# XinMing0411/AC-VAE

Hardware: AMD Instinct MI355X
Metric: train-step captions/s (and audio-sec/s) at B=32, 1/2/4/8 MI355X (higher is better)
Workload: dtype f32

## Files before the change

### acvae_amd/csrc/conv.h

```cpp
#pragma once
#include <hip/hip_runtime.h>
#include <stdint.h>
#include "common.h"
#include "job_table.h"

struct DropoutSpec {
  float p;
  const uint8_t* mask;
  uint64_t seed;
  uint32_t site;
};

enum { UP_PLAIN = 0, UP_POOL = 1, UP_DROP = 2 };

namespace acvae {
int conv3x3_igemm(const float* X, const float* scale, const float* shift, const float* Wp, float* Y, float* partials,
                  int N, int H, int W, int Cin, int Cout, hipStream_t st);
int conv_partials_rows(int N, int H, int W);
int conv3x3_igemm_bf16(const bf16_t* X, const float* scale, const float* shift, const bf16_t* Wp, bf16_t* Y,
                       float* partials, int N, int H, int W, int Cin, int Cout, hipStream_t st);
long conv3x3_wgrad_bf16_slab_floats(int N, int H, int W, int Cin, int Cout);
int conv3x3_wgrad_bf16_splits(int N, int H, int W, int Cin, int Cout);
int conv3x3_wgrad_bf16_launch(const bf16_t* dY, const bf16_t* X, const float* scale, const float* shift, float* slab, int N,
                              int H, int W, int Cin, int Cout, hipStream_t st);
int wgrad_reduce(const float* slab, int nsplit, float* dW_oihw, int Cout, int Cin, hipStream_t st);
long conv3x3_wgrad_slab_floats(int N, int H, int W, int Cin, int Cout);
int conv3x3_wgrad(const float* dY, const float* X, const float* scale, const float* shift, float* dW_oihw, float* slab,
                  int N, int H, int W, int Cin, int Cout, hipStream_t st);
bool conv3x3_wino_ok(int H, int W, int Cin, int Cout);
long conv3x3_wino_weight_floats(int Cin, int Cout);
int conv_wino_partials_rows(int N, int H, int W);
int conv3x3_wino_weights(const float* W_oihw, float* U, int Cout, int Cin, bool dgrad, hipStream_t st);
struct WinoWeightsJob { const float* W; float* U; int Cout, Cin, dgrad; };
using WinoWeightsBatch = RangeTable<WinoWeightsJob, 32>;
int conv3x3_wino_weights_batch(WinoWeightsBatch& b, hipStream_t st);
struct WinoBnReduce { const float* Y; const float* scale; const float* shift; const float* mean; const float* invstd; };
int conv3x3_wino(const float* X, const float* scale, const float* shift, const float* U, float* Y, float* partials, int N,
                 int H, int W, int Cin, int Cout, hipStream_t st, const WinoBnReduce* red = nullptr);
bool conv3x3_wino_wgrad_ok(int H, int W, int Cin, int Cout);
long conv3x3_wino_wgrad_slab_floats(int N, int H, int W, int Cin, int Cout);
int conv3x3_wino_wgrad(const float* dY, const float* X, const float* scale, const float* shift, float* dW_oihw, float* slab,
                       int N, int H, int W, int Cin, int Cout, hipStream_t st);
template <class T>
int repack_weights(const float* W_oihw, T* Wf, T* Wd, int Cout, int Cin, hipStream_t st);
struct RepackJob { const float* W; void* dst; int Cout, Cin, dgrad; };
using RepackBatch = RangeTable<RepackJob, 32>;
template <class T>
int repack_weights_batch(RepackBatch& b, hipStream_t st);
inline int conv3x3_igemm(const bf16_t* X, const float* scale, const float* shift, const bf16_t* Wp, bf16_t* Y,
                         float* partials, int N, int H, int W, int Cin, int Cout, hipStream_t st) {
  return conv3x3_igemm_bf16(X, scale, shift, Wp, Y, partials, N, H, W, Cin, Cout, st);
}
inline int conv3x3_wgrad(const bf16_t* dY, const bf16_t* X, const float* scale, const float* shift, float* dW_oihw,
                         float* slab, int N, int H, int W, int Cin, int Cout, hipStream_t st) {
  int r = conv3x3_wgrad_bf16_launch(dY, X, scale, shift, slab, N, H, W, Cin, Cout, st);
  if (r != 0) return r;
  return wgrad_reduce(slab, conv3x3_wgrad_bf16_splits(N, H, W, Cin, Cout), dW_oihw, Cout, Cin, st);
}
template <class T>
inline long conv3x3_wgrad_slab_floats_t(int N, int H, int W, int Cin, int Cout) {
  return sizeof(T) == 2 ? conv3x3_wgrad_bf16_slab_floats(N, H, W, Cin, Cout) : conv3x3_wgrad_slab_floats(N, H, W, Cin, Cout);
}
int bn0_stats(const float* x, float* partials, long rows, int F, int* nparts, hipStream_t st);
int bn0_partials_rows(long rows);
int bn_finalize(const float* partials, int P, int C, double count, const float* gamma, const float* beta,
                float* running_mean, float* running_var, int64_t* nbt, int training, float* scale, float* shift,
                float* mean, float* invstd, double* dpart, hipStream_t st);
long colsum_scratch_doubles(int width);
int colsum_tickets_reset(double* dpart, hipStream_t st);
long colsum_ticket_words();
int colsum2(const float* x, int P, int width, double* dpart, float* out, float* out2, int split, hipStream_t st);
struct ColsumJob { const float* x; int P, width; float* out; float* out_b; int R; long d0; };
using ColsumBatch = RangeTable<ColsumJob, 6, int>;
int colsum_batch(ColsumBatch& b, double* dpart, long dpart_doubles, hipStream_t st);
bool colsum_batch_plan(ColsumBatch& b, long dpart_doubles, long* dsum_doubles);
int conv1_first_blocks(int N, int T);
template <class TY>
int conv1_first_fwd(const float* x, const float* scale0, const float* shift0, const float* W1, TY* Y,
                    float* partials, int N, int T, int F, hipStream_t st);
template <class TY>
int conv1_first_bwd(const float* x, const float* scale0, const float* shift0, const float* mean0, const float* invstd0,
                    const float* W1, const TY* dY, float* dw_part, float* bn_part, float* dW1, float* dgamma0,
                    float* dbeta0, double* dpart, int N, int T, int F, hipStream_t st);
template <class T>
int bn_relu_pool(const T* Y, const float* scale, const float* shift, T* P, int N, int H, int W, int C,
                 DropoutSpec drop, hipStream_t st, bool pool = true);
int bn_bwd_blocks(int N, int H, int W, int C);
template <class T>
int bn_bwd(const T* Y, const T* dO, int upstream, const float* scale, const float* shift, const float* mean,
           const float* invstd, float* partials, float* sum_g, float* sum_gy, T* dY, double* dpart, int N, int H,
           int W, int C, DropoutSpec drop, hipStream_t st, bool batch_stats = true, int ready_rows = 0);
template <class T>
int relu_mask(const T* Y, const float* scale, const float* shift, uint8_t* out, int N, int H, int W, int C, hipStream_t st);
template <class T>
int freq_mean(const T* P, float* out, long rows, int Fp, int C, hipStream_t st);
template <class T>
int freq_mean_bwd(const float* dae, T* dP, long rows, int Fp, int C, hipStream_t st);
int time_pool(const float* ae, float* out, int N, int S, int C, DropoutSpec drop, hipStream_t st);
int relu_dropout(float* x, int total, DropoutSpec drop, hipStream_t st);
}

int acvae_gemm_nt_dual(const float* A1, int64_t lda1, const float* B1, int64_t ldb1, int K1, const float* A2,
                       int64_t lda2, const float* B2, int64_t ldb2, int K2, const float* bias, float* C, int64_t ldc,
                       int M, int N, int accumulate, hipStream_t st, float* skws = nullptr);
int acvae_gemm_nt_pair(const float* A0, int64_t lda0, const float* B0, int64_t ldb0, int K0, const float* bias0, float* C0,
                       int64_t ldc0, int N0, int acc0, const float* A1, int64_t lda1, const float* B1, int64_t ldb1, int K1,
                       const float* bias1, float* C1, int64_t ldc1, int N1, int acc1, int M, hipStream_t st);
constexpr int TN_TICKETS = 256;
int acvae_gemm_tn_fused(const float* A, int64_t lda, const float* B, int64_t ldb, float* C, int64_t ldc, int M, int N, int K,
                        int accumulate, float* ws, int64_t ws_bytes, hipStream_t st);
long acvae_skinny_ws_floats();
long acvae_skinny_ticket_words();
int acvae_skinny_ws_reset(float* ws, hipStream_t st);
struct TransposeJob { const float* in; long ld_in; float* out; long ld_out; int rows, cols; };
using TransposeBatch = acvae::RangeTable<TransposeJob, 12, int>;
int acvae_transpose_batch(TransposeBatch& b, hipStream_t st);
```

### acvae_amd/csrc/conv.hip

```cpp
#include "mfma_tile.h"
#include "../../include/acvae_hip.h"
#include "conv.h"
#include "prof.h"

namespace {
using namespace mfma;

struct FastDiv {
  unsigned long long mul;
  static FastDiv make(int d) { return FastDiv{((1ULL << 40) + (unsigned long long)d - 1) / (unsigned long long)d}; }
  __device__ __forceinline__ int div(int x) const { return (int)(((unsigned long long)(unsigned)x * mul) >> 40); }
};

struct ConvKMajorLoader {
  const float* X;
  const float* scale;
  const float* shift;
  int H, W, C, M, NC;
  FastDiv dW, dH;
  int dy, dx, ci;
  bool colok;
  float4 sc, sh;
  template <int WT>
  __device__ __forceinline__ void init(int col0) {
// ... 422 lines not shown
        acc[0][1] = __builtin_amdgcn_mfma_f32_32x32x2f32(af.x, bp.y, acc[0][1], 0, 0, 0);
        acc[0][2] = __builtin_amdgcn_mfma_f32_32x32x2f32(af.x, bc, acc[0][2], 0, 0, 0);
        acc[1][0] = __builtin_amdgcn_mfma_f32_32x32x2f32(af.y, bp.x, acc[1][0], 0, 0, 0);
        acc[1][1] = __builtin_amdgcn_mfma_f32_32x32x2f32(af.y, bp.y, acc[1][1], 0, 0, 0);
        acc[1][2] = __builtin_amdgcn_mfma_f32_32x32x2f32(af.y, bc, acc[1][2], 0, 0, 0);
      }
    }
    if (ks + 1 < nk) stash(cur ^ 1);
    __syncthreads();
  }
  float* Cw = EM == 2 ? Cs : slab + (long)(2 * z + wm) * Cout * NC;
#pragma unroll
  for (int em = 0; em < 2; ++em)
#pragma unroll
    for (int r = 0; r < 16; ++r) {
      const int rho = (r & 3) + 8 * (r >> 2) + 4 * lh;
      const int m = row0 + (EM == 2 ? wm * 64 : 0) + 2 * rho + em;
      if (m >= Cout) continue;
      float* out = Cw + (long)m * NC + dyi * 3 * C + c0;
      out[2 * wn * C + 2 * li + 0] = acc[em][0][r];
      out[2 * wn * C + 2 * li + 1] = acc[em][1][r];
      out[C + wn * 32 + li] = acc[em][2][r];
    }
}

__global__ void wgrad_reduce_kernel(const float* __restrict__ slab, int nsplit, float* __restrict__ dW, int Cout,
                                    int Cin) {
  const long total = (long)Cout * 9 * Cin;
  for (long i = blockIdx.x * (long)blockDim.x + threadIdx.x; i < total; i += (long)gridDim.x * blockDim.x) {
    float a0 = 0.f, a1 = 0.f, a2 = 0.f, a3 = 0.f;
    int z = 0;
    for (; z + 3 < nsplit; z += 4) {
      a0 += slab[(long)z * total + i]; a1 += slab[(long)(z + 1) * total + i];
      a2 += slab[(long)(z + 2) * total + i]; a3 += slab[(long)(z + 3) * total + i];
    }
    for (; z < nsplit; ++z) a0 += slab[(long)z * total + i];
    const float acc = (a0 + a1) + (a2 + a3);
    const int co = (int)(i / (9 * Cin)), rem = (int)(i % (9 * Cin));
    const int tap = rem / Cin, ci = rem % Cin;
    dW[((long)co * Cin + ci) * 9 + tap] = acc;
  }
}

template <class T>
__global__ void repack_fwd_kernel(const float* __restrict__ W, T* __restrict__ Wf, int Cout, int Cin) {
  const long total = (long)Cout * Cin * 9;
  for (long i = blockIdx.x * (long)blockDim.x + threadIdx.x; i < total; i += (long)gridDim.x * blockDim.x) {
    const int co = (int)(i / (9 * Cin)), rem = (int)(i % (9 * Cin));
    const int tap = rem / Cin, ci = rem % Cin;
    Wf[i] = (T)W[((long)co * Cin + ci) * 9 + tap];
  }
}
template <class T>
__global__ void repack_dgrad_kernel(const float* __restrict__ W, T* __restrict__ Wd, int Cout, int Cin) {
  const long total = (long)Cout * Cin * 9;
  for (long i = blockIdx.x * (long)blockDim.x + threadIdx.x; i < total; i += (long)gridDim.x * blockDim.x) {
    const int ci = (int)(i / (9 * Cout)), rem = (int)(i % (9 * Cout));
    const int tp = rem / Cout, co = rem % Cout;
    Wd[i] = (T)W[((long)co * Cin + ci) * 9 + (8 - tp)];
  }
}

template <class T>
__global__ void repack_batch_kernel(acvae::RepackBatch b) {
  const long total = b.start[b.n];
  for (long i = blockIdx.x * (long)blockDim.x + threadIdx.x; i < total; i += (long)gridDim.x * blockDim.x) {
    const int l = b.find(i);
    const acvae::RepackJob& job = b.job[l];
    const long k = i - b.start[l];
    const int Cout = job.Cout, Cin = job.Cin;
    const float* W = job.W;
    T* out = reinterpret_cast<T*>(job.dst);
    if (!job.dgrad) {
      const int co = (int)(k / (9 * Cin)), rem = (int)(k % (9 * Cin));
      const int tap = rem / Cin, ci = rem % Cin;
      out[k] = (T)W[((long)co * Cin + ci) * 9 + tap];
    } else {
      const int ci = (int)(k / (9 * Cout)), rem = (int)(k % (9 * Cout));
      const int tp = rem / Cout, co = rem % Cout;
      out[k] = (T)W[((long)co * Cin + ci) * 9 + (8 - tp)];
    }
  }
}

__global__ __launch_bounds__(256) void bn0_stats_kernel(const float* __restrict__ x, float* __restrict__ partials,
                                                        long rows, int F, int rows_per_block) {
  __shared__ float red[2][4][64];
  const int w = threadIdx.x & 63, g = threadIdx.x >> 6;
  const long r0 = (long)blockIdx.x * rows_per_block;
  float s = 0.f, q = 0.f;
  if (w < F)
    for (long r = r0 + g; r < r0 + rows_per_block && r < rows; r += 4) {
      const float v = x[r * F + w];
      s += v; q += v * v;
    }
  red[0][g][w] = s; red[1][g][w] = q;
  __syncthreads();
  if (threadIdx.x < 64 && w < F) {
    float* out = partials + (long)blockIdx.x * 2 * F;
    out[w] = red[0][0][w] + red[0][1][w] + red[0][2][w] + red[0][3][w];
    out[F + w] = red[1][0][w] + red[1][1][w] + red[1][2][w] + red[1][3][w];
  }
}

constexpr int CS_R = 64;
constexpr int CS_TICKETS = 128;
inline int cs_groups(int P) { return P < 1 ? 1 : P < 16 ? P : P <= 1024 ? 16 : P <= 4096 ? 32 : CS_R; }

struct BnFinalizeArgs {
  double count;
  const float *gamma, *beta;
  float *running_mean, *running_var;
  int64_t* nbt;
  float *scale, *shift, *mean_out, *invstd_out;
};

__device__ __forceinline__ void cs_store(double* p, double v) {
  __hip_atomic_store(reinterpret_cast<unsigned long long*>(p), (unsigned long long)__double_as_longlong(v), __ATOMIC_RELAXED,
                     __HIP_MEMORY_SCOPE_AGENT);
}
__device__ __forceinline__ double cs_load(const double* p) {
  return __longlong_as_double((long long)__hip_atomic_load(reinterpret_cast<const unsigned long long*>(p), __ATOMIC_RELAXED,
                                                           __HIP_MEMORY_SCOPE_AGENT));
}
__device__ __forceinline__ bool cs_last_arriver(unsigned* ticket, unsigned expect, int* s_last) {
  asm volatile("s_waitcnt vmcnt(0)" ::: "memory");
  __syncthreads();
  if (threadIdx.x == 0) {
    const unsigned prev = __hip_atomic_fetch_add(ticket, 1u, __ATOMIC_RELAXED, __HIP_MEMORY_SCOPE_AGENT);
    const int last = prev == expect - 1u;
    if (last) __hip_atomic_store(ticket, 0u, __ATOMIC_RELAXED, __HIP_MEMORY_SCOPE_AGENT);
    *s_last = last;
  }
  __syncthreads();
  return *s_last != 0;
}

template <bool FINALIZE>
__global__ __launch_bounds__(256) void colsum_kernel(const float* __restrict__ partials, int P, int width, double* __restrict__ dpart,
                                                     float* __restrict__ out, float* __restrict__ out2, int split,
                                                     BnFinalizeArgs bn) {
  __shared__ double red[4][64];
  __shared__ int s_last;
  unsigned* tickets = reinterpret_cast<unsigned*>(dpart);
  double* dsum = dpart + CS_TICKETS / 2;
  const int il = threadIdx.x & 63, g = threadIdx.x >> 6;
  const int i = blockIdx.x * 64 + il;
  const int R = gridDim.y;
  double a = 0.0;
  if (i < width)
    for (int p = blockIdx.y + g * R; p < P; p += 4 * R) a += (double)partials[(long)p * width + i];
  red[g][il] = a;
  __syncthreads();
  if (g == 0 && i < width) cs_store(dsum + (long)blockIdx.y * width + i, red[0][il] + red[1][il] + red[2][il] + red[3][il]);
  if (!FINALIZE) {
    if (!cs_last_arriver(tickets + blockIdx.x, (unsigned)R, &s_last)) return;
    if (g != 0 || i >= width) return;
    double t = 0.0;
    for (int r0 = 0; r0 < R; r0 += 8) {
      double v[8];
#pragma unroll
      for (int u = 0; u < 8; ++u) v[u] = r0 + u < R ? cs_load(dsum + (long)(r0 + u) * width + i) : 0.0;
#pragma unroll
      for (int u = 0; u < 8; ++u)
        if (r0 + u < R) t += v[u];
    }
    if (split > 0 && i >= split) out2[i - split] = (float)t;
    else out[i] = (float)t;
  } else {
    const int C = width >> 1, cb = C >> 6;
    const int xc = blockIdx.x % cb;
    if (!cs_last_arriver(tickets + xc, (unsigned)(2 * R), &s_last)) return;
    if (g != 0) return;
    const int c = xc * 64 + il;
    double sm = 0.0, q = 0.0;
    for (int r0 = 0; r0 < R; r0 += 8) {
      double v[8], w[8];
#pragma unroll
      for (int u = 0; u < 8; ++u) {
        v[u] = r0 + u < R ? cs_load(dsum + (long)(r0 + u) * width + c) : 0.0;
        w[u] = r0 + u < R ? cs_load(dsum + (long)(r0 + u) * width + C + c) : 0.0;
      }
#pragma unroll
      for (int u = 0; u < 8; ++u)
        if (r0 + u < R) { sm += v[u]; q += w[u]; }
    }
    const double mean = sm / bn.count;
    double var = q / bn.count - mean * mean;
    if (var < 0.0) var = 0.0;
    const float invstd = (float)(1.0 / sqrt(var + 1e-5));
    const float sc = bn.gamma[c] * invstd;
    bn.scale[c] = sc; bn.shift[c] = bn.beta[c] - (float)mean * sc;
    bn.mean_out[c] = (float)mean; bn.invstd_out[c] = invstd;
    const double unbiased = bn.count > 1.0 ? var * bn.count / (bn.count - 1.0) : var;
    bn.running_mean[c] = 0.9f * bn.running_mean[c] + 0.1f * (float)mean;
    bn.running_var[c] = 0.9f * bn.running_var[c] + 0.1f * (float)unbiased;
    if (c == 0 && bn.nbt) bn.nbt[0] += 1;
  }
}

__global__ __launch_bounds__(256) void colsum_batch_kernel(acvae::ColsumBatch b, double* __restrict__ dpart) {
  __shared__ double red[4][64];
  __shared__ int s_last;
  const int j = b.find((int)blockIdx.x);
  const acvae::ColsumJob& job = b.job[j];
  const int R = job.R;
  if ((int)blockIdx.y >= R) return;
  const float* __restrict__ partials = job.x;
  const int P = job.P, width = job.width;
  unsigned* tickets = reinterpret_cast<unsigned*>(dpart);
  double* dsum = dpart + CS_TICKETS / 2 + job.d0;
  const int il = threadIdx.x & 63, g = threadIdx.x >> 6;
  const int i = ((int)blockIdx.x - b.start[j]) * 64 + il;
  double a = 0.0;
  if (i < width)
    for (int p = blockIdx.y + g * R; p < P; p += 4 * R) a += (double)partials[(long)p * width + i];
  red[g][il] = a;
  __syncthreads();
  if (g == 0 && i < width) cs_store(dsum + (long)blockIdx.y * width + i, red[0][il] + red[1][il] + red[2][il] + red[3][il]);
  if (!cs_last_arriver(tickets + blockIdx.x, (unsigned)R, &s_last)) return;
  if (g != 0 || i >= width) return;
  double t = 0.0;
  for (int r0 = 0; r0 < R; r0 += 8) {
    double v[8];
#pragma unroll
    for (int u = 0; u < 8; ++u) v[u] = r0 + u < R ? cs_load(dsum + (long)(r0 + u) * width + i) : 0.0;
#pragma unroll
    for (int u = 0; u < 8; ++u)
      if (r0 + u < R) t += v[u];
  }
  job.out[i] = (float)t;
  if (job.out_b) job.out_b[i] = (float)t;
}

__global__ __launch_bounds__(64) void bn_eval_kernel(int C, const float* __restrict__ gamma, const float* __restrict__ beta,
                                                     const float* __restrict__ running_mean, const float* __restrict__ running_var,
                                                     float* __restrict__ scale, float* __restrict__ shift,
                                                     float* __restrict__ mean_out, float* __restrict__ invstd_out) {
  const int c = blockIdx.x * 64 + threadIdx.x;
  if (c >= C) return;
  const float invstd = 1.0f / sqrtf(running_var[c] + 1e-5f);
  const float sc = gamma[c] * invstd;
  scale[c] = sc; shift[c] = beta[c] - running_mean[c] * sc;
  mean_out[c] = running_mean[c]; invstd_out[c] = invstd;
}

constexpr int C1_RB = 8;
template <class TY>
__global__ __launch_bounds__(256) void conv1_first_fwd_kernel(const float* __restrict__ x,
                                                              const float* __restrict__ scale0,
                                                              const float* __restrict__ shift0,
                                                              const float* __restrict__ W1, TY* __restrict__ Y,
                                                              float* __restrict__ partials, int T, int F) {
  __shared__ float wl[64 * 9];
  __shared__ float patch[(C1_RB + 2) * 66];
  __shared__ float red[2][16][64];
  const int nblk_t = (T + C1_RB - 1) / C1_RB;
  const int n = blockIdx.x / nblk_t, t0 = (blockIdx.x % nblk_t) * C1_RB;
  for (int i = threadIdx.x; i < 64 * 9; i += 256) wl[i] = W1[i];
  for (int i = threadIdx.x; i < (C1_RB + 2) * 66; i += 256) {
    const int r = i / 66, cidx = i % 66;
    const int t = t0 + r - 1, w = cidx - 1;
    float v = 0.f;
    if (t >= 0 && t < T && w >= 0 && w < F) v = x[((long)n * T + t) * F + w] * scale0[w] + shift0[w];
    patch[i] = v;
  }
  __syncthreads();
  const int cq = threadIdx.x & 15, pp = threadIdx.x >> 4;
  float wreg[4][9];
#pragma unroll
  for (int c = 0; c < 4; ++c)
#pragma unroll
    for (int k = 0; k < 9; ++k) wreg[c][k] = wl[(cq * 4 + c) * 9 + k];
  float s[4] = {0, 0, 0, 0}, q[4] = {0, 0, 0, 0};
  for (int pix = pp; pix < C1_RB * 64; pix += 16) {
    const int r = pix >> 6, w = pix & 63;
    const int t = t0 + r;
    if (t >= T || w >= F) continue;
    float in[9];
#pragma unroll
    for (int k = 0; k < 9; ++k) in[k] = patch[(r + k / 3) * 66 + w + k % 3];
    float o[4];
#pragma unroll
    for (int c = 0; c < 4; ++c) {
      float a = 0.f;
#pragma unroll
      for (int k = 0; k < 9; ++k) a += wreg[c][k] * in[k];
      if (!std::is_same<TY, float>::value) a = round_bf16(a);
      o[c] = a; s[c] += a; q[c] += a * a;
    }
    store4(Y + (((long)n * T + t) * F + w) * 64 + cq * 4, make_float4(o[0], o[1], o[2], o[3]));
  }
#pragma unroll
  for (int c = 0; c < 4; ++c) { red[0][pp][cq * 4 + c] = s[c]; red[1][pp][cq * 4 + c] = q[c]; }
  __syncthreads();
  if (partials && threadIdx.x < 128) {
    const int which = threadIdx.x >> 6, co = threadIdx.x & 63;
    float a = 0.f;
    for (int i = 0; i < 16; ++i) a += red[which][i][co];
    partials[(long)blockIdx.x * 128 + which * 64 + co] = a;
  }
}

template <class TY>
__global__ __launch_bounds__(256) void conv1_first_bwd_kernel(const float* __restrict__ x,
                                                              const float* __restrict__ scale0,
                                                              const float* __restrict__ shift0,
                                                              const float* __restrict__ mean0,
                                                              const float* __restrict__ invstd0,
                                                              const float* __restrict__ W1,
                                                              const TY* __restrict__ dY,
                                                              float* __restrict__ dw_part, float* __restrict__ bn_part,
                                                              int T, int F) {
  __shared__ float wl[64 * 9];
  __shared__ float patch[(C1_RB + 2) * 66];
  constexpr int D_FLOATS = (C1_RB + 2) * 64 * 9, WACC_FLOATS = 8 * 576;
  __shared__ float scratch[D_FLOATS > WACC_FLOATS ? D_FLOATS : WACC_FLOATS];
  float* D = scratch;
  float (*wacc)[576] = reinterpret_cast<float (*)[576]>(scratch);
  const int nblk_t = (T + C1_RB - 1) / C1_RB;
  const int n = blockIdx.x / nblk_t, t0 = (blockIdx.x % nblk_t) * C1_RB;
  for (int i = threadIdx.x; i < 64 * 9; i += 256) wl[i] = W1[i];
  for (int i = threadIdx.x; i < (C1_RB + 2) * 66; i += 256) {
    const int r = i / 66, cidx = i % 66;
    const int t = t0 + r - 1, w = cidx - 1;
    float v = 0.f;
    if (t >= 0 && t < T && w >= 0 && w < F) v = x[((long)n * T + t) * F + w] * scale0[w] + shift0[w];
    patch[i] = v;
  }
  __syncthreads();
  const int cq = threadIdx.x & 15, pp = threadIdx.x >> 4;
  float wreg[4][9];
#pragma unroll
  for (int c = 0; c < 4; ++c)
#pragma unroll
    for (int k = 0; k < 9; ++k) wreg[c][k] = wl[(cq * 4 + c) * 9 + k];
  float dwacc[4][9];
#pragma unroll
  for (int c = 0; c < 4; ++c)
#pragma unroll
    for (int k = 0; k < 9; ++k) dwacc[c][k] = 0.f;
  constexpr int C1_IT = (C1_RB + 2) * 64 / 16, C1_UN = 4;
  static_assert(C1_IT % C1_UN == 0, "pixel loop is unrolled by four");
  auto fetch = [&](int it, float4& g) {
    const int pix = pp + it * 16;
    const int r = pix >> 6, w = pix & 63;
    const int t = t0 + r - 1;
    g = make_float4(0.f, 0.f, 0.f, 0.f);
    if (t >= 0 && t < T && w < F) g = load4(dY + (((long)n * T + t) * F + w) * 64 + cq * 4);
  };
  float4 gq[C1_UN], gn[C1_UN];
#pragma unroll
  for (int u = 0; u < C1_UN; ++u) fetch(u, gq[u]);
  for (int it0 = 0; it0 < C1_IT; it0 += C1_UN) {
    if (it0 + C1_UN < C1_IT) {
#pragma unroll
      for (int u = 0; u < C1_UN; ++u) fetch(it0 + C1_UN + u, gn[u]);
    }
#pragma unroll
    for (int u = 0; u < C1_UN; ++u) {
      const int pix = pp + (it0 + u) * 16;
      const int r = pix >> 6, w = pix & 63;
      const int t = t0 + r - 1;
      const bool inimg = (t >= 0 && t < T && w < F);
      const float gv[4] = {gq[u].x, gq[u].y, gq[u].z, gq[u].w};
      float d[9];
#pragma unroll
      for (int k = 0; k < 9; ++k) d[k] = gv[0] * wreg[0][k] + gv[1] * wreg[1][k] + gv[2] * wreg[2][k] + gv[3] * wreg[3][k];
#pragma unroll
      for (int k = 0; k < 9; ++k) d[k] = row16_sum(d[k]);
      if (cq == 0) {
#pragma unroll
        for (int k = 0; k < 9; ++k) D[(r * 64 + w) * 9 + k] = d[k];
      }
      if (inimg && r >= 1 && r <= C1_RB) {
#pragma unroll
        for (int k = 0; k < 9; ++k) {
          const float in = patch[(r - 1 + k / 3) * 66 + w + k % 3];
#pragma unroll
          for (int c = 0; c < 4; ++c) dwacc[c][k] += gv[c] * in;
        }
      }
    }
#pragma unroll
    for (int u = 0; u < C1_UN; ++u) gq[u] = gn[u];
  }
  __syncthreads();
  const int w = threadIdx.x & 63, rr = threadIdx.x >> 6;
  float sg = 0.f, sgx = 0.f;
  if (w < F)
    for (int r = rr; r < C1_RB; r += 4) {
      const int t = t0 + r;
      if (t >= T) break;
      float dx = 0.f;
#pragma unroll
      for (int k = 0; k < 9; ++k) {
        const int dy = k / 3 - 1, dxx = k % 3 - 1;
        const int pr = r + 1 - dy, pw2 = w - dxx;
        if (pw2 >= 0 && pw2 < 64) dx += D[(pr * 64 + pw2) * 9 + k];
      }
      const float xhat = (x[((long)n * T + t) * F + w] - mean0[w]) * invstd0[w];
      sg += dx; sgx += dx * xhat;
    }
  float asum[3] = {0.f, 0.f, 0.f};
#pragma unroll
  for (int half = 0; half < 2; ++half) {
    __syncthreads();
    if ((pp >> 3) == half) {
#pragma unroll
      for (int c = 0; c < 4; ++c)
#pragma unroll
        for (int k = 0; k < 9; ++k) wacc[pp & 7][cq * 36 + c * 9 + k] = dwacc[c][k];
    }
    __syncthreads();
#pragma unroll
    for (int q = 0; q < 3; ++q) {
      const int i = threadIdx.x + q * 256;
      if (i < 576)
        for (int j = 0; j < 8; ++j) asum[q] += wacc[j][i];
    }
  }
#pragma unroll
  for (int q = 0; q < 3; ++q) {
    const int i = threadIdx.x + q * 256;
    if (i < 576) dw_part[(long)blockIdx.x * 576 + i] = asum[q];
  }
  __syncthreads();
  float* rb = scratch;
  rb[rr * 128 + w] = sg; rb[rr * 128 + 64 + w] = sgx;
  __syncthreads();
  if (threadIdx.x < 128) {
    const int which = threadIdx.x >> 6, ww = threadIdx.x & 63;
    bn_part[(long)blockIdx.x * 128 + which * 64 + ww] =
        rb[0 * 128 + which * 64 + ww] + rb[1 * 128 + which * 64 + ww] + rb[2 * 128 + which * 64 + ww] +
        rb[3 * 128 + which * 64 + ww];
  }
}

__device__ __forceinline__ float4 bnrelu4(float4 v, float4 sc, float4 sh) {
  return make_float4(fmaxf(v.x * sc.x + sh.x, 0.f), fmaxf(v.y * sc.y + sh.y, 0.f), fmaxf(v.z * sc.z + sh.z, 0.f),
                     fmaxf(v.w * sc.w + sh.w, 0.f));
}
__device__ __forceinline__ float4 drop4(const DropoutSpec& d, long idx4, int n, int ho, int wo, int c, int Ho, int Wo,
                                        int C) {
  if (d.p <= 0.f) return make_float4(1.f, 1.f, 1.f, 1.f);
  const float k = 1.0f / (1.0f - d.p);
  if (d.mask) {
    const long b = (((long)n * C + c) * Ho + ho) * Wo + wo;
    const long cs = (long)Ho * Wo;
    return make_float4(d.mask[b] ? k : 0.f, d.mask[b + cs] ? k : 0.f, d.mask[b + 2 * cs] ? k : 0.f,
                       d.mask[b + 3 * cs] ? k : 0.f);
  }
  const uint4 r = philox4x32(d.seed, (uint64_t)idx4, d.site);
  const float u = 1.0f / 16777216.0f;
  return make_float4((float)(r.x >> 8) * u >= d.p ? k : 0.f, (float)(r.y >> 8) * u >= d.p ? k : 0.f,
                     (float)(r.z >> 8) * u >= d.p ? k : 0.f, (float)(r.w >> 8) * u >= d.p ? k : 0.f);
}

template <class T>
__global__ void bn_relu_pool_kernel(const T* __restrict__ Y, const float* __restrict__ scale,
                                    const float* __restrict__ shift, T* __restrict__ P, int N, int H, int W, int C,
                                    DropoutSpec drop) {
  const int Ho = H / 2, Wo = W / 2, C4 = C / 4;
  const long total = (long)N * Ho * Wo * C4;
  for (long i = blockIdx.x * (long)blockDim.x + threadIdx.x; i < total; i += (long)gridDim.x * blockDim.x) {
    const int c4 = (int)(i % C4);
    long r = i / C4;
    const int wo = (int)(r % Wo); r /= Wo;
    const int ho = (int)(r % Ho);
    const int n = (int)(r / Ho);
    const float4 sc = *reinterpret_cast<const float4*>(scale + c4 * 4);
    const float4 sh = *reinterpret_cast<const float4*>(shift + c4 * 4);
    const T* y = Y + ((((long)n * H + 2 * ho) * W + 2 * wo) * C + c4 * 4);
    const float4 a = bnrelu4(load4(y), sc, sh);
    const float4 b = bnrelu4(load4(y + C), sc, sh);
    const float4 c = bnrelu4(load4(y + (long)W * C), sc, sh);
    const float4 d = bnrelu4(load4(y + (long)W * C + C), sc, sh);
    const float4 m = drop4(drop, i, n, ho, wo, c4 * 4, Ho, Wo, C);
    float4 o;
    o.x = ((a.x + b.x + c.x + d.x) * 0.25f) * m.x; o.y = ((a.y + b.y + c.y + d.y) * 0.25f) * m.y;
    o.z = ((a.z + b.z + c.z + d.z) * 0.25f) * m.z; o.w = ((a.w + b.w + c.w + d.w) * 0.25f) * m.w;
    store4(P + 4 * i, o);
  }
}

template <class T>
__global__ void bn_relu_drop_kernel(const T* __restrict__ Y, const float* __restrict__ scale,
                                    const float* __restrict__ shift, T* __restrict__ P, int N, int H, int W, int C,
                                    DropoutSpec drop) {
  const int C4 = C / 4;
  const long total = (long)N * H * W * C4;
  for (long i = blockIdx.x * (long)blockDim.x + threadIdx.x; i < total; i += (long)gridDim.x * blockDim.x) {
    const int c4 = (int)(i % C4);
    long r = i / C4;
    const int w = (int)(r % W); r /= W;
    const int h = (int)(r % H);
    const int n = (int)(r / H);
    const float4 sc = *reinterpret_cast<const float4*>(scale + c4 * 4);
    const float4 sh = *reinterpret_cast<const float4*>(shift + c4 * 4);
    const float4 a = bnrelu4(load4(Y + 4 * i), sc, sh);
    const float4 m = drop4(drop, i, n, h, w, c4 * 4, H, W, C);
    store4(P + 4 * i, make_float4(a.x * m.x, a.y * m.y, a.z * m.z, a.w * m.w));
  }
}

template <class T>
__global__ void relu_mask_kernel(const T* __restrict__ Y, const float* __restrict__ scale,
                                 const float* __restrict__ shift, uint8_t* __restrict__ out, int N, int H, int W, int C) {
  const long total = (long)N * H * W * C;
  for (long i = blockIdx.x * (long)blockDim.x + threadIdx.x; i < total; i += (long)gridDim.x * blockDim.x) {
    const int c = (int)(i % C);
    long r = i / C;
    const int w = (int)(r % W); r /= W;
    const int h = (int)(r % H);
    const int n = (int)(r / H);
    const float y = load1(Y + i);
    out[(((long)n * C + c) * H + h) * W + w] = (y * scale[c] + shift[c] <= 0.f) ? 0 : 1;
  }
}

template <int UP, class T>
__device__ __forceinline__ float4 upstream4(const T* __restrict__ dO, const DropoutSpec& drop, int n, int h, int w,
                                            int c, int H, int W, int C) {
  if (UP == UP_PLAIN) return load4(dO + ((((long)n * H + h) * W + w) * C + c));
  if (UP == UP_DROP) {
    const long i4 = ((((long)n * H + h) * W + w) * C + c) >> 2;
    float4 v = load4(dO + 4 * i4);
    const float4 m = drop4(drop, i4, n, h, w, c, H, W, C);
    v.x *= m.x; v.y *= m.y; v.z *= m.z; v.w *= m.w;
    return v;
  }
  const int Ho = H / 2, Wo = W / 2;
  const int ho = h >> 1, wo = w >> 1;
  if (ho >= Ho || wo >= Wo) return make_float4(0.f, 0.f, 0.f, 0.f);
  const long i4 = ((((long)n * Ho + ho) * Wo + wo) * C + c) >> 2;
  float4 v = load4(dO + 4 * i4);
  const float4 m = drop4(drop, i4, n, ho, wo, c, Ho, Wo, C);
  v.x *= m.x * 0.25f; v.y *= m.y * 0.25f; v.z *= m.z * 0.25f; v.w *= m.w * 0.25f;
  return v;
}

template <int UP, class T>
__global__ __launch_bounds__(256) void bn_bwd_reduce_kernel(const T* __restrict__ Y, const T* __restrict__ dO,
                                                            const float* __restrict__ scale,
                                                            const float* __restrict__ shift,
                                                            const float* __restrict__ mean,
                                                            const float* __restrict__ invstd,
                                                            float* __restrict__ partials, int N, int H, int W, int C,
                                                            int pix_per_block, DropoutSpec drop) {
  extern __shared__ float red[];
  const int Cc = C < 1024 ? C : 1024;
  const int C4 = Cc / 4;
  const int cq = threadIdx.x % C4, pl = threadIdx.x / C4, npl = 256 / C4;
  const long M = (long)N * H * W;
  const long p0 = (long)blockIdx.x * pix_per_block;
  const int c = blockIdx.y * Cc + cq * 4;
  float s[4] = {0, 0, 0, 0}, q[4] = {0, 0, 0, 0};
  if (pl < npl) {
    const float4 sc = *reinterpret_cast<const float4*>(scale + c), sh = *reinterpret_cast<const float4*>(shift + c);
    const float4 mu = *reinterpret_cast<const float4*>(mean + c), is = *reinterpret_cast<const float4*>(invstd + c);
    for (long p = p0 + pl; p < p0 + pix_per_block && p < M; p += npl) {
      int w = 0, h = 0, n = 0;
      if (UP != UP_PLAIN) {
        w = (int)(p % W);
        const long t = p / W;
        h = (int)(t % H); n = (int)(t / H);
      }
      const float4 y = load4(Y + p * C + c);
      float4 g = UP == UP_PLAIN ? load4(dO + p * C + c) : upstream4<UP>(dO, drop, n, h, w, c, H, W, C);
      if (y.x * sc.x + sh.x <= 0.f) g.x = 0.f;
      if (y.y * sc.y + sh.y <= 0.f) g.y = 0.f;
      if (y.z * sc.z + sh.z <= 0.f) g.z = 0.f;
      if (y.w * sc.w + sh.w <= 0.f) g.w = 0.f;
      s[0] += g.x; s[1] += g.y; s[2] += g.z; s[3] += g.w;
      q[0] += g.x * ((y.x - mu.x) * is.x); q[1] += g.y * ((y.y - mu.y) * is.y);
      q[2] += g.z * ((y.z - mu.z) * is.z); q[3] += g.w * ((y.w - mu.w) * is.w);
    }
  }
#pragma unroll
  for (int k = 0; k < 4; ++k) { red[k * 256 + threadIdx.x] = s[k]; red[(4 + k) * 256 + threadIdx.x] = q[k]; }
  __syncthreads();
  if (threadIdx.x < C4) {
    float a[8] = {0, 0, 0, 0, 0, 0, 0, 0};
    for (int j = 0; j < npl; ++j)
#pragma unroll
      for (int k = 0; k < 8; ++k) a[k] += red[k * 256 + j * C4 + threadIdx.x];
    float* out = partials + (long)blockIdx.x * 2 * C;
#pragma unroll
    for (int k = 0; k < 4; ++k) { out[c + k] = a[k]; out[C + c + k] = a[4 + k]; }
  }
}

template <int UP, class T>
__global__ void bn_bwd_apply_kernel(const T* __restrict__ Y, const T* __restrict__ dO,
                                    const float* __restrict__ scale, const float* __restrict__ shift,
                                    const float* __restrict__ mean, const float* __restrict__ invstd,
                                    const float* __restrict__ sum_g, const float* __restrict__ sum_gy,
                                    T* __restrict__ dYout, int N, int H, int W, int C, DropoutSpec drop,
                                    int batch_stats) {
  const int C4 = C / 4;
  const long total = (long)N * H * W * C4;
  const float invn = batch_stats ? 1.0f / (float)((long)N * H * W) : 0.f;
  for (long i = blockIdx.x * (long)blockDim.x + threadIdx.x; i < total; i += (long)gridDim.x * blockDim.x) {
    const int c = (int)(i % C4) * 4;
    const long p = i / C4;
    const int w = (int)(p % W);
    const long t = p / W;
    const int h = (int)(t % H), n = (int)(t / H);
    const float4 sc = *reinterpret_cast<const float4*>(scale + c), sh = *reinterpret_cast<const float4*>(shift + c);
    const float4 mu = *reinterpret_cast<const float4*>(mean + c), is = *reinterpret_cast<const float4*>(invstd + c);
    const float4 sg = *reinterpret_cast<const float4*>(sum_g + c), sgy = *reinterpret_cast<const float4*>(sum_gy + c);
    const float4 y = load4(Y + 4 * i);
    float4 g = upstream4<UP>(dO, drop, n, h, w, c, H, W, C);
    if (y.x * sc.x + sh.x <= 0.f) g.x = 0.f;
    if (y.y * sc.y + sh.y <= 0.f) g.y = 0.f;
    if (y.z * sc.z + sh.z <= 0.f) g.z = 0.f;
    if (y.w * sc.w + sh.w <= 0.f) g.w = 0.f;
    float4 o;
    o.x = sc.x * (g.x - sg.x * invn - ((y.x - mu.x) * is.x) * (sgy.x * invn));
    o.y = sc.y * (g.y - sg.y * invn - ((y.y - mu.y) * is.y) * (sgy.y * invn));
    o.z = sc.z * (g.z - sg.z * invn - ((y.z - mu.z) * is.z) * (sgy.z * invn));
    o.w = sc.w * (g.w - sg.w * invn - ((y.w - mu.w) * is.w) * (sgy.w * invn));
    store4(dYout + 4 * i, o);
  }
}

template <class T>
__global__ __launch_bounds__(256) void bn_bwd_apply_plain_kernel(const T* __restrict__ Y, const T* __restrict__ dO,
                                                                 const float* __restrict__ scale, const float* __restrict__ shift,
                                                                 const float* __restrict__ mean, const float* __restrict__ invstd,
                                                                 const float* __restrict__ sum_g, const float* __restrict__ sum_gy,
                                                                 T* __restrict__ dYout, long total, int C4, float invn) {
  const long tid = blockIdx.x * 256L + threadIdx.x, stride = gridDim.x * 256L;
  const int c = (int)(tid % C4) * 4;
  const float4 sc = *reinterpret_cast<const float4*>(scale + c), sh = *reinterpret_cast<const float4*>(shift + c);
  const float4 mu = *reinterpret_cast<const float4*>(mean + c), is = *reinterpret_cast<const float4*>(invstd + c);
  float4 a = *reinterpret_cast<const float4*>(sum_g + c), b = *reinterpret_cast<const float4*>(sum_gy + c);
  a.x *= invn; a.y *= invn; a.z *= invn; a.w *= invn;
  b.x *= invn; b.y *= invn; b.z *= invn; b.w *= invn;
  auto one = [&](float4 y, float4 g) {
    if (y.x * sc.x + sh.x <= 0.f) g.x = 0.f;
    if (y.y * sc.y + sh.y <= 0.f) g.y = 0.f;
    if (y.z * sc.z + sh.z <= 0.f) g.z = 0.f;
    if (y.w * sc.w + sh.w <= 0.f) g.w = 0.f;
    float4 o;
    o.x = sc.x * (g.x - a.x - ((y.x - mu.x) * is.x) * b.x);
    o.y = sc.y * (g.y - a.y - ((y.y - mu.y) * is.y) * b.y);
    o.z = sc.z * (g.z - a.z - ((y.z - mu.z) * is.z) * b.z);
    o.w = sc.w * (g.w - a.w - ((y.w - mu.w) * is.w) * b.w);
    return o;
  };
  long i = tid;
  for (; i + stride < total; i += 2 * stride) {
    const float4 y0 = load4(Y + 4 * i), g0 = load4(dO + 4 * i);
    const float4 y1 = load4(Y + 4 * (i + stride)), g1 = load4(dO + 4 * (i + stride));
    store4(dYout + 4 * i, one(y0, g0));
    store4(dYout + 4 * (i + stride), one(y1, g1));
  }
  if (i < total) store4(dYout + 4 * i, one(load4(Y + 4 * i), load4(dO + 4 * i)));
}

struct PoolIdx { int n, ho, wo, c4; };
__device__ __forceinline__ PoolIdx pool_idx(unsigned i, unsigned C4, unsigned Wc, unsigned Hc) {
  PoolIdx r;
  r.c4 = (int)(i % C4);
  unsigned t = i / C4;
  r.wo = (int)(t % Wc); t /= Wc;
  r.ho = (int)(t % Hc);
  r.n = (int)(t / Hc);
  return r;
}
template <class T>
__device__ __forceinline__ float4 pool_upstream(const T* __restrict__ dO, const DropoutSpec& drop, const PoolIdx& q, int Ho, int Wo,
                                                int C) {
  if (q.ho >= Ho || q.wo >= Wo) return make_float4(0.f, 0.f, 0.f, 0.f);
  const long i4 = ((((long)q.n * Ho + q.ho) * Wo + q.wo) * C + q.c4 * 4) >> 2;
  float4 v = load4(dO + 4 * i4);
  const float4 m = drop4(drop, i4, q.n, q.ho, q.wo, q.c4 * 4, Ho, Wo, C);
  v.x *= m.x * 0.25f; v.y *= m.y * 0.25f; v.z *= m.z * 0.25f; v.w *= m.w * 0.25f;
  return v;
}
template <class T>
__global__ __launch_bounds__(256) void bn_bwd_apply_pool_kernel(const T* __restrict__ Y, const T* __restrict__ dO,
                                                                const float* __restrict__ scale, const float* __restrict__ shift,
                                                                const float* __restrict__ mean, const float* __restrict__ invstd,
                                                                const float* __restrict__ sum_g, const float* __restrict__ sum_gy,
                                                                T* __restrict__ dYout, int N, int H, int W, int C, DropoutSpec drop,
                                                                float invn) {
  const int C4 = C / 4, Ho = H / 2, Wo = W / 2, Hc = (H + 1) / 2, Wc = (W + 1) / 2;
  const unsigned total = (unsigned)N * Hc * Wc * C4;
  for (unsigned i = blockIdx.x * 256u + threadIdx.x; i < total; i += gridDim.x * 256u) {
    const PoolIdx q = pool_idx(i, C4, Wc, Hc);
    const int c = q.c4 * 4;
    const float4 sc = *reinterpret_cast<const float4*>(scale + c), sh = *reinterpret_cast<const float4*>(shift + c);
    const float4 mu = *reinterpret_cast<const float4*>(mean + c), is = *reinterpret_cast<const float4*>(invstd + c);
    float4 a = *reinterpret_cast<const float4*>(sum_g + c), b = *reinterpret_cast<const float4*>(sum_gy + c);
    a.x *= invn; a.y *= invn; a.z *= invn; a.w *= invn;
    b.x *= invn; b.y *= invn; b.z *= invn; b.w *= invn;
    const long base = (((long)q.n * H + 2 * q.ho) * W + 2 * q.wo) * C + c;
    const bool hx = 2 * q.ho + 1 < H, wx = 2 * q.wo + 1 < W;
    const long off[4] = {0, (long)C, (long)W * C, (long)W * C + C};
    const bool ok[4] = {true, wx, hx, hx && wx};
    float4 y[4];
#pragma unroll
    for (int k = 0; k < 4; ++k) y[k] = ok[k] ? load4(Y + base + off[k]) : make_float4(0.f, 0.f, 0.f, 0.f);
    const float4 gp = pool_upstream(dO, drop, q, Ho, Wo, C);
#pragma unroll
    for (int k = 0; k < 4; ++k) {
      if (!ok[k]) continue;
      float4 g = gp;
      if (y[k].x * sc.x + sh.x <= 0.f) g.x = 0.f;
      if (y[k].y * sc.y + sh.y <= 0.f) g.y = 0.f;
      if (y[k].z * sc.z + sh.z <= 0.f) g.z = 0.f;
      if (y[k].w * sc.w + sh.w <= 0.f) g.w = 0.f;
      float4 o;
      o.x = sc.x * (g.x - a.x - ((y[k].x - mu.x) * is.x) * b.x);
      o.y = sc.y * (g.y - a.y - ((y[k].y - mu.y) * is.y) * b.y);
      o.z = sc.z * (g.z - a.z - ((y[k].z - mu.z) * is.z) * b.z);
      o.w = sc.w * (g.w - a.w - ((y[k].w - mu.w) * is.w) * b.w);
      store4(dYout + base + off[k], o);
    }
  }
}
template <class T>
__global__ __launch_bounds__(256) void bn_bwd_reduce_pool_kernel(const T* __restrict__ Y, const T* __restrict__ dO,
                                                                 const float* __restrict__ scale, const float* __restrict__ shift,
                                                                 const float* __restrict__ mean, const float* __restrict__ invstd,
                                                                 float* __restrict__ partials, int N, int H, int W, int C,
                                                                 int win_per_block, DropoutSpec drop) {
  extern __shared__ float red[];
  const int Cc = C < 1024 ? C : 1024;
  const int C4 = Cc / 4, Ho = H / 2, Wo = W / 2;
  const int cq = threadIdx.x % C4, pl = threadIdx.x / C4, npl = 256 / C4;
  const unsigned M = (unsigned)N * Ho * Wo;
  const unsigned p0 = blockIdx.x * (unsigned)win_per_block;
  const int c = blockIdx.y * Cc + cq * 4;
  float s[4] = {0, 0, 0, 0}, qv[4] = {0, 0, 0, 0};
  if (pl < npl) {
    const float4 sc = *reinterpret_cast<const float4*>(scale + c), sh = *reinterpret_cast<const float4*>(shift + c);
    const float4 mu = *reinterpret_cast<const float4*>(mean + c), is = *reinterpret_cast<const float4*>(invstd + c);
    for (unsigned p = p0 + pl; p < p0 + win_per_block && p < M; p += npl) {
      PoolIdx q;
      q.c4 = c >> 2;
      q.wo = (int)(p % (unsigned)Wo);
      const unsigned t = p / (unsigned)Wo;
      q.ho = (int)(t % (unsigned)Ho); q.n = (int)(t / (unsigned)Ho);
      const long base = (((long)q.n * H + 2 * q.ho) * W + 2 * q.wo) * C + c;
      const float4 y0 = load4(Y + base), y1 = load4(Y + base + C), y2 = load4(Y + base + (long)W * C),
                   y3 = load4(Y + base + (long)W * C + C);
      const float4 gp = pool_upstream(dO, drop, q, Ho, Wo, C);
      const float4 ys[4] = {y0, y1, y2, y3};
#pragma unroll
      for (int k = 0; k < 4; ++k) {
        float4 g = gp;
        const float4 y = ys[k];
        if (y.x * sc.x + sh.x <= 0.f) g.x = 0.f;
        if (y.y * sc.y + sh.y <= 0.f) g.y = 0.f;
        if (y.z * sc.z + sh.z <= 0.f) g.z = 0.f;
        if (y.w * sc.w + sh.w <= 0.f) g.w = 0.f;
        s[0] += g.x; s[1] += g.y; s[2] += g.z; s[3] += g.w;
        qv[0] += g.x * ((y.x - mu.x) * is.x); qv[1] += g.y * ((y.y - mu.y) * is.y);
        qv[2] += g.z * ((y.z - mu.z) * is.z); qv[3] += g.w * ((y.w - mu.w) * is.w);
      }
    }
  }
#pragma unroll
  for (int k = 0; k < 4; ++k) { red[k * 256 + threadIdx.x] = s[k]; red[(4 + k) * 256 + threadIdx.x] = qv[k]; }
  __syncthreads();
  if (threadIdx.x < C4) {
    float a[8] = {0, 0, 0, 0, 0, 0, 0, 0};
    for (int j = 0; j < npl; ++j)
#pragma unroll
      for (int k = 0; k < 8; ++k) a[k] += red[k * 256 + j * C4 + threadIdx.x];
    float* out = partials + (long)blockIdx.x * 2 * C;
#pragma unroll
    for (int k = 0; k < 4; ++k) { out[c + k] = a[k]; out[C + c + k] = a[4 + k]; }
  }
}

template <class T>
__global__ void freq_mean_kernel(const T* __restrict__ P, float* __restrict__ out, long rows, int Fp, int C) {
  const long total = rows * C;
  for (long i = blockIdx.x * (long)blockDim.x + threadIdx.x; i < total; i += (long)gridDim.x * blockDim.x) {
    const long r = i / C;
    const int c = (int)(i % C);
    float a = 0.f;
    for (int f = 0; f < Fp; ++f) a += load1(P + (r * Fp + f) * C + c);
    out[i] = a / (float)Fp;
  }
}
template <class T>
__global__ void freq_mean_bwd_kernel(const float* __restrict__ dae, T* __restrict__ dP, long rows, int Fp, int C) {
  const long total = rows * Fp * C;
  const float k = 1.0f / (float)Fp;
  for (long i = blockIdx.x * (long)blockDim.x + threadIdx.x; i < total; i += (long)gridDim.x * blockDim.x) {
    const int c = (int)(i % C);
    const long r = i / ((long)Fp * C);
    dP[i] = (T)(dae[r * C + c] * k);
  }
}
__global__ void time_pool_kernel(const float* __restrict__ ae, float* __restrict__ out, int N, int S, int C,
                                 DropoutSpec drop) {
  const int total = N * C;
  for (int i = blockIdx.x * blockDim.x + threadIdx.x; i < total; i += gridDim.x * blockDim.x) {
    const int n = i / C, c = i % C;
    float mx = -INFINITY, sm = 0.f;
    for (int s = 0; s < S; ++s) {
      const float v = ae[((long)n * S + s) * C + c];
      mx = fmaxf(mx, v); sm += v;
    }
    float o = mx + sm / (float)S;
    if (drop.p > 0.f) {
      const float k = 1.0f / (1.0f - drop.p);
      const bool keep = drop.mask ? drop.mask[i] != 0 : dropout_keep(drop.seed, drop.site, (uint64_t)i, drop.p);
      o = keep ? o * k : 0.f;
    }
    out[i] = o;
  }
}
__global__ void relu_dropout_kernel(float* __restrict__ x, int total, DropoutSpec drop) {
  for (int i = blockIdx.x * blockDim.x + threadIdx.x; i < total; i += gridDim.x * blockDim.x) {
    float o = fmaxf(x[i], 0.f);
    if (drop.p > 0.f) {
      const float k = 1.0f / (1.0f - drop.p);
      const bool keep = drop.mask ? drop.mask[i] != 0 : dropout_keep(drop.seed, drop.site, (uint64_t)i, drop.p);
      o = keep ? o * k : 0.f;
    }
    x[i] = o;
  }
}

inline int ew_grid(long n) {
  long b = (n + 255) / 256;
  return (int)(b < 1 ? 1 : (b > 8192 ? 8192 : b));
}

}

namespace acvae {

constexpr int CONV_BMT = 128;

int conv3x3_igemm(const float* X, const float* scale, const float* shift, const float* Wp, float* Y, float* partials,
                  int N, int H, int W, int Cin, int Cout, hipStream_t st) {
  if (!X || !Wp || !Y) return ACVAE_EINVAL;
  if (Cin % 32 != 0 || Cout % 4 != 0) return ACVAE_EUNSUPPORTED;
  if (!aligned16(X) || !aligned16(Wp) || !aligned16(Y)) return ACVAE_EALIGN;
  const int M = N * H * W, K = 9 * Cin;
  ConvStatsEpilogue ep{Y, partials, Cout};
  prof_begin(ACVAE_PROF_CONV_IGEMM, st);
  ConvStripLoader al{X, scale, shift, H, W, Cin, M};
  const int bn = Cout <= 64 ? 64 : 128;
  const dim3 grid(cdiv(M, CV_BMT), cdiv(Cout, bn)), block(nt_threads<CV_BMT>());
  const bool dma = Cout % bn == 0;
  if (bn == 64) {
    if (dma) hipLaunchKernelGGL((conv_igemm3_kernel<64, true>), grid, block, 0, st, al, Wp, ep, M, Cout, K);
    else hipLaunchKernelGGL((conv_igemm3_kernel<64, false>), grid, block, 0, st, al, Wp, ep, M, Cout, K);
  } else {
    if (dma) hipLaunchKernelGGL((conv_igemm3_kernel<128, true>), grid, block, 0, st, al, Wp, ep, M, Cout, K);
    else hipLaunchKernelGGL((conv_igemm3_kernel<128, false>), grid, block, 0, st, al, Wp, ep, M, Cout, K);
  }
  prof_end(ACVAE_PROF_CONV_IGEMM, st);
  ACVAE_LAUNCH_CHECK();
  return ACVAE_OK;
}
int conv_partials_rows(int N, int H, int W) { return cdiv((long)N * H * W, CONV_BMT); }

static bool wgrad_strip(int NC, int Cout) { (void)Cout; return NC % 576 == 0; }
static int wgrad_slabs_per_slice(int NC, int Cout) { return wgrad_strip(NC, Cout) && Cout <= 64 ? 2 : 1; }
static int wgrad_splits(int M, int Cout, int NC) {
  const bool narrow = Cout <= 64, w192 = wgrad_strip(NC, Cout);
  const long tiles = w192 ? (long)cdiv(Cout, narrow ? 64 : 128) * (NC / 192)
                          : (long)cdiv(Cout, narrow ? 64 : 128) * cdiv(NC, narrow ? 256 : 128);
  const long slots = 256L * (wgrad_strip(NC, Cout) ? 3 : ((w192 ? !narrow : narrow) ? 3 : 4));
  const int maxs = cdiv(M, 16 * BKT) & ~7;
  const double t_mfma = 2.0 * (double)M * Cout * NC / 1.1e14;
  const double t_slab = 2.0 * (double)Cout * NC * 4.0 / 0.67e12 * wgrad_slabs_per_slice(NC, Cout);
  int best = 8;
  double best_t = 1e30;
  for (int k = 8; k <= (maxs < 8 ? 8 : maxs) && tiles * k <= 5 * slots; k += 8) {
    const long b = tiles * k;
    const double fill = (double)b / (double)(slots * ((b + slots - 1) / slots));
    const double t = t_mfma / (2 * b < 3 * slots ? fill * 0.75 : fill) + k * t_slab;
    if (t < best_t) { best_t = t; best = k; }
  }
  return best;
}
long conv3x3_wgrad_slab_floats(int N, int H, int W, int Cin, int Cout) {
  return (long)wgrad_splits(N * H * W, Cout, 9 * Cin) * wgrad_slabs_per_slice(9 * Cin, Cout) * Cout * 9 * Cin;
}
int conv3x3_wgrad(const float* dY, const float* X, const float* scale, const float* shift, float* dW_oihw, float* slab,
                  int N, int H, int W, int Cin, int Cout, hipStream_t st) {
  if (!dY || !X || !dW_oihw || !slab) return ACVAE_EINVAL;
  if (Cin % 4 != 0 || Cout % 4 != 0) return ACVAE_EUNSUPPORTED;
  const int M = N * H * W, NC = 9 * Cin;
  const int s = wgrad_splits(M, Cout, NC);
  const int k_per = cdiv(cdiv(M, s), BKT) * BKT;
  if ((long)(M + 4096) * (W > H ? W : H) >= (1L << 40)) return ACVAE_EUNSUPPORTED;
  ConvKMajorLoader bl{X, scale, shift, H, W, Cin, M, NC, FastDiv::make(W), FastDiv::make(H)};
  prof_begin(ACVAE_PROF_CONV_WGRAD, st);
  if (wgrad_strip(NC, Cout)) {
    const FastDiv fw = FastDiv::make(W), fh = FastDiv::make(H);
    if (Cout <= 64) {
      dim3 grid(cdiv(Cout, 64), NC / 192, s);
      hipLaunchKernelGGL((conv_wgrad3_kernel<1>), grid, dim3(256), 0, st, dY, X, scale, shift, slab, M, Cout, H, W, Cin,
                         fw, fh, k_per);
    } else {
      dim3 grid(cdiv(Cout, 128), NC / 192, s);
      hipLaunchKernelGGL((conv_wgrad3_kernel<2>), grid, dim3(256), 0, st, dY, X, scale, shift, slab, M, Cout, H, W, Cin,
                         fw, fh, k_per);
    }
  } else if (Cout <= 64) {
    dim3 grid(cdiv(Cout, 64), cdiv(NC, 256), s);
    hipLaunchKernelGGL((conv_wgrad_kernel<1, 4>), grid, dim3(256), 0, st, dY, bl, slab, M, Cout, NC, k_per);
  } else {
    dim3 grid(cdiv(Cout, 128), cdiv(NC, 128), s);
    hipLaunchKernelGGL((conv_wgrad_kernel<2, 2>), grid, dim3(256), 0, st, dY, bl, slab, M, Cout, NC, k_per);
  }
  prof_end(ACVAE_PROF_CONV_WGRAD, st);
  hipLaunchKernelGGL(wgrad_reduce_kernel, dim3(ew_grid((long)Cout * NC)), dim3(256), 0, st, slab,
                     s * wgrad_slabs_per_slice(NC, Cout), dW_oihw, Cout, Cin);
  ACVAE_LAUNCH_CHECK();
  return ACVAE_OK;
}

int wgrad_reduce(const float* slab, int nsplit, float* dW_oihw, int Cout, int Cin, hipStream_t st) {
  hipLaunchKernelGGL(wgrad_reduce_kernel, dim3(ew_grid((long)Cout * 9 * Cin)), dim3(256), 0, st, slab, nsplit, dW_oihw, Cout,
                     Cin);
  ACVAE_LAUNCH_CHECK();
  return ACVAE_OK;
}

template <class T>
int repack_weights(const float* W_oihw, T* Wf, T* Wd, int Cout, int Cin, hipStream_t st) {
  const long total = (long)Cout * Cin * 9;
  if (Wf) hipLaunchKernelGGL(repack_fwd_kernel<T>, dim3(ew_grid(total)), dim3(256), 0, st, W_oihw, Wf, Cout, Cin);
  if (Wd) hipLaunchKernelGGL(repack_dgrad_kernel<T>, dim3(ew_grid(total)), dim3(256), 0, st, W_oihw, Wd, Cout, Cin);
  ACVAE_LAUNCH_CHECK();
  return ACVAE_OK;
}
template int repack_weights<float>(const float*, float*, float*, int, int, hipStream_t);
template int repack_weights<bf16_t>(const float*, bf16_t*, bf16_t*, int, int, hipStream_t);
template <class T>
int repack_weights_batch(RepackBatch& b, hipStream_t st) {
  if (!b.ok()) return ACVAE_EINVAL;
  if (b.n <= 0) return ACVAE_OK;
  for (int l = 0; l < b.n; ++l)
    if (!b.job[l].W || !b.job[l].dst) return ACVAE_EINVAL;
  const long total = b.seal([](const RepackJob& j) { return (long)j.Cout * j.Cin * 9; });
  hipLaunchKernelGGL(repack_batch_kernel<T>, dim3(cdiv(total, 256) > 8192 ? 8192 : cdiv(total, 256)), dim3(256), 0, st, b);
  ACVAE_LAUNCH_CHECK();
  return ACVAE_OK;
}
template int repack_weights_batch<float>(RepackBatch&, hipStream_t);
template int repack_weights_batch<bf16_t>(RepackBatch&, hipStream_t);

int bn0_stats(const float* x, float* partials, long rows, int F, int* nparts, hipStream_t st) {
  if (F > 64) return ACVAE_EUNSUPPORTED;
  const int rpb = 256;
  const int nb = cdiv(rows, rpb);
  hipLaunchKernelGGL(bn0_stats_kernel, dim3(nb), dim3(256), 0, st, x, partials, rows, F, rpb);
  *nparts = nb;
  ACVAE_LAUNCH_CHECK();
  return ACVAE_OK;
}
int bn0_partials_rows(long rows) { return cdiv(rows, 256); }

int colsum2(const float* partials, int P, int width, double* dpart, float* out, float* out2, int split,
            hipStream_t st) {
  if (cdiv(width, 64) > CS_TICKETS) return ACVAE_EUNSUPPORTED;
  const int R = cs_groups(P);
  hipLaunchKernelGGL(colsum_kernel<false>, dim3(cdiv(width, 64), R), dim3(256), 0, st, partials, P, width, dpart, out, out2, split,
                     BnFinalizeArgs{});
  ACVAE_LAUNCH_CHECK();
  return ACVAE_OK;
}
bool colsum_batch_plan(ColsumBatch& b, long dpart_doubles, long* dsum_doubles) {
  long d = 0;
  for (int j = 0; j < b.n; ++j) {
    ColsumJob& c = b.job[j];
    c.R = cs_groups(c.P);
    c.d0 = d;
    d += (long)c.R * c.width;
  }
  const int blocks = b.seal([](const ColsumJob& c) { return cdiv(c.width, 64); });
  if (dsum_doubles) *dsum_doubles = d;
  return !(b.n == 1 || blocks > CS_TICKETS || CS_TICKETS / 2 + d > dpart_doubles);
}
int colsum_batch(ColsumBatch& b, double* dpart, long dpart_doubles, hipStream_t st) {
  if (!b.ok()) return ACVAE_EINVAL;
  if (b.n <= 0) return ACVAE_OK;
  if (!colsum_batch_plan(b, dpart_doubles, nullptr)) {
    for (int j = 0; j < b.n; ++j) {
      const ColsumJob& c = b.job[j];
      ACVAE_TRY(colsum2(c.x, c.P, c.width, dpart, c.out, nullptr, 0, st));
      if (c.out_b) ACVAE_TRY(colsum2(c.x, c.P, c.width, dpart, c.out_b, nullptr, 0, st));
    }
    return ACVAE_OK;
  }
  int maxr = 1;
  for (int j = 0; j < b.n; ++j)
    if (b.job[j].R > maxr) maxr = b.job[j].R;
  hipLaunchKernelGGL(colsum_batch_kernel, dim3(b.start[b.n], maxr), dim3(256), 0, st, b, dpart);
  ACVAE_LAUNCH_CHECK();
  return ACVAE_OK;
}
long colsum_scratch_doubles(int width) { return CS_TICKETS / 2 + (long)CS_R * width; }
long colsum_ticket_words() { return CS_TICKETS; }
int colsum_tickets_reset(double* dpart, hipStream_t st) {
  return hipMemsetAsync(dpart, 0, CS_TICKETS * sizeof(unsigned), st) == hipSuccess ? ACVAE_OK : (int)hipGetLastError();
}

int bn_finalize(const float* partials, int P, int C, double count, const float* gamma, const float* beta,
                float* running_mean, float* running_var, int64_t* nbt, int training, float* scale, float* shift,
                float* mean, float* invstd, double* dpart, hipStream_t st) {
  if (training) {
    if (C % 64 != 0 || cdiv(2 * C, 64) > CS_TICKETS) return ACVAE_EUNSUPPORTED;
    const int R = cs_groups(P);
    hipLaunchKernelGGL(colsum_kernel<true>, dim3(2 * C / 64, R), dim3(256), 0, st, partials, P, 2 * C, dpart, nullptr, nullptr, 0,
                       BnFinalizeArgs{count, gamma, beta, running_mean, running_var, nbt, scale, shift, mean, invstd});
  } else {
    hipLaunchKernelGGL(bn_eval_kernel, dim3(cdiv(C, 64)), dim3(64), 0, st, C, gamma, beta, running_mean, running_var, scale,
                       shift, mean, invstd);
  }
  ACVAE_LAUNCH_CHECK();
  return ACVAE_OK;
}

int conv1_first_blocks(int N, int T) { return N * cdiv(T, C1_RB); }
template <class TY>
int conv1_first_fwd(const float* x, const float* scale0, const float* shift0, const float* W1, TY* Y,
                    float* partials, int N, int T, int F, hipStream_t st) {
  if (F != 64) return ACVAE_EUNSUPPORTED;
  hipLaunchKernelGGL(conv1_first_fwd_kernel<TY>, dim3(conv1_first_blocks(N, T)), dim3(256), 0, st, x, scale0, shift0, W1,
                     Y, partials, T, F);
  ACVAE_LAUNCH_CHECK();
  return ACVAE_OK;
}
template int conv1_first_fwd<float>(const float*, const float*, const float*, const float*, float*, float*, int, int, int, hipStream_t);
template int conv1_first_fwd<bf16_t>(const float*, const float*, const float*, const float*, bf16_t*, float*, int, int, int, hipStream_t);
template <class TY>
int conv1_first_bwd(const float* x, const float* scale0, const float* shift0, const float* mean0, const float* invstd0,
                    const float* W1, const TY* dY, float* dw_part, float* bn_part, float* dW1, float* dgamma0,
                    float* dbeta0, double* dpart, int N, int T, int F, hipStream_t st) {
  if (F != 64) return ACVAE_EUNSUPPORTED;
  const int nb = conv1_first_blocks(N, T);
  hipLaunchKernelGGL(conv1_first_bwd_kernel<TY>, dim3(nb), dim3(256), 0, st, x, scale0, shift0, mean0, invstd0, W1, dY,
                     dw_part, bn_part, T, F);
  ACVAE_TRY(colsum2(dw_part, nb, 576, dpart, dW1, nullptr, 0, st));
  ACVAE_TRY(colsum2(bn_part, nb, 128, dpart, dbeta0, dgamma0, 64, st));
  return ACVAE_OK;
}
template int conv1_first_bwd<float>(const float*, const float*, const float*, const float*, const float*, const float*, const float*, float*, float*, float*, float*, float*, double*, int, int, int, hipStream_t);
template int conv1_first_bwd<bf16_t>(const float*, const float*, const float*, const float*, const float*, const float*, const bf16_t*, float*, float*, float*, float*, float*, double*, int, int, int, hipStream_t);

template <class T>
int bn_relu_pool(const T* Y, const float* scale, const float* shift, T* P, int N, int H, int W, int C,
                 DropoutSpec drop, hipStream_t st, bool pool) {
  const long total = pool ? (long)N * (H / 2) * (W / 2) * (C / 4) : (long)N * H * W * (C / 4);
  if (total <= 0 || C % 4 != 0) return ACVAE_EINVAL;
  if (pool)
    hipLaunchKernelGGL(bn_relu_pool_kernel<T>, dim3(ew_grid(total)), dim3(256), 0, st, Y, scale, shift, P, N, H, W, C, drop);
  else
    hipLaunchKernelGGL(bn_relu_drop_kernel<T>, dim3(ew_grid(total)), dim3(256), 0, st, Y, scale, shift, P, N, H, W, C, drop);
  ACVAE_LAUNCH_CHECK();
  return ACVAE_OK;
}
template int bn_relu_pool<float>(const float*, const float*, const float*, float*, int, int, int, int, DropoutSpec, hipStream_t, bool);
template int bn_relu_pool<bf16_t>(const bf16_t*, const float*, const float*, bf16_t*, int, int, int, int, DropoutSpec, hipStream_t, bool);

static int bnb_pix(int C) {
  const int Cc = C < 1024 ? C : 1024;
  const int npl = 256 / (Cc / 4) > 0 ? 256 / (Cc / 4) : 1;
  return npl * 32 < 32 ? 32 : npl * 32;
}
int bn_bwd_blocks(int N, int H, int W, int C) { return cdiv((long)N * H * W, bnb_pix(C)); }
template <class T>
int bn_bwd(const T* Y, const T* dO, int upstream, const float* scale, const float* shift, const float* mean,
           const float* invstd, float* partials, float* sum_g, float* sum_gy, T* dY, double* dpart, int N, int H,
           int W, int C, DropoutSpec drop, hipStream_t st, bool batch_stats, int ready_rows) {
  const int Cc = C < 1024 ? C : 1024;
  if (C % 4 != 0 || 1024 % Cc != 0 || C % Cc != 0) return ACVAE_EUNSUPPORTED;
  if (ready_rows > 0 && upstream != UP_PLAIN) return ACVAE_EINVAL;
  const dim3 rgrid(bn_bwd_blocks(N, H, W, C), C / Cc);
  const int nb = rgrid.x;
  const size_t shm = 256 * 8 * sizeof(float);
  const long total = (long)N * H * W * (C / 4);
#define BN_BWD_LAUNCH(UP_)                                                                                             \
  hipLaunchKernelGGL((bn_bwd_reduce_kernel<UP_, T>), rgrid, dim3(256), shm, st, Y, dO, scale, shift, mean, invstd, partials, \
                     N, H, W, C, bnb_pix(C), drop);                                                                       \
  ACVAE_TRY(colsum2(partials, nb, 2 * C, dpart, sum_g, sum_gy, C, st));         \
  hipLaunchKernelGGL((bn_bwd_apply_kernel<UP_, T>), dim3(ew_grid(total)), dim3(256), 0, st, Y, dO, scale, shift, mean,  \
                     invstd, sum_g, sum_gy, dY, N, H, W, C, drop, batch_stats ? 1 : 0)
  const float invn = batch_stats ? 1.0f / (float)((long)N * H * W) : 0.f;
  const bool small = (long)N * H * W * C < (1L << 31);
  if (upstream == UP_POOL && small && H >= 2 && W >= 2) {
    const long wins = (long)N * (H / 2) * (W / 2);
    const int wpb = bnb_pix(C) / 4 > 0 ? bnb_pix(C) / 4 : 1;
    const dim3 pgrid((unsigned)cdiv(wins, wpb), C / Cc);
    hipLaunchKernelGGL((bn_bwd_reduce_pool_kernel<T>), pgrid, dim3(256), shm, st, Y, dO, scale, shift, mean, invstd, partials, N, H, W,
                       C, wpb, drop);
    ACVAE_TRY(colsum2(partials, (int)pgrid.x, 2 * C, dpart, sum_g, sum_gy, C, st));
    const long totalp = (long)N * ((H + 1) / 2) * ((W + 1) / 2) * (C / 4);
    hipLaunchKernelGGL((bn_bwd_apply_pool_kernel<T>), dim3(ew_grid(totalp)), dim3(256), 0, st, Y, dO, scale, shift, mean, invstd,
                       sum_g, sum_gy, dY, N, H, W, C, drop, invn);
  } else if (upstream == UP_POOL) { BN_BWD_LAUNCH(UP_POOL); }
  else if (upstream == UP_DROP) { BN_BWD_LAUNCH(UP_DROP); }
  else {
    if (ready_rows <= 0)
      hipLaunchKernelGGL((bn_bwd_reduce_kernel<UP_PLAIN, T>), rgrid, dim3(256), shm, st, Y, dO, scale, shift, mean, invstd, partials,
                         N, H, W, C, bnb_pix(C), drop);
    ACVAE_TRY(colsum2(partials, ready_rows > 0 ? ready_rows : nb, 2 * C, dpart, sum_g, sum_gy, C, st));
    int g = ew_grid((total + 1) / 2);
    if ((C / 4) > 256 && (g & 1)) ++g;
    if ((256L * g) % (C / 4) == 0)
      hipLaunchKernelGGL((bn_bwd_apply_plain_kernel<T>), dim3(g), dim3(256), 0, st, Y, dO, scale, shift, mean, invstd, sum_g, sum_gy,
                         dY, total, C / 4, invn);
    else
      hipLaunchKernelGGL((bn_bwd_apply_kernel<UP_PLAIN, T>), dim3(ew_grid(total)), dim3(256), 0, st, Y, dO, scale, shift, mean,
                         invstd, sum_g, sum_gy, dY, N, H, W, C, drop, batch_stats ? 1 : 0);
  }
#undef BN_BWD_LAUNCH
  ACVAE_LAUNCH_CHECK();
  return ACVAE_OK;
}
template int bn_bwd<float>(const float*, const float*, int, const float*, const float*, const float*, const float*, float*, float*, float*, float*, double*, int, int, int, int, DropoutSpec, hipStream_t, bool, int);
template int bn_bwd<bf16_t>(const bf16_t*, const bf16_t*, int, const float*, const float*, const float*, const float*, float*, float*, float*, bf16_t*, double*, int, int, int, int, DropoutSpec, hipStream_t, bool, int);

template <class T>
int relu_mask(const T* Y, const float* scale, const float* shift, uint8_t* out, int N, int H, int W, int C, hipStream_t st) {
  hipLaunchKernelGGL(relu_mask_kernel<T>, dim3(ew_grid((long)N * H * W * C)), dim3(256), 0, st, Y, scale, shift, out, N, H, W, C);
  ACVAE_LAUNCH_CHECK();
  return ACVAE_OK;
}
template int relu_mask<float>(const float*, const float*, const float*, uint8_t*, int, int, int, int, hipStream_t);
template int relu_mask<bf16_t>(const bf16_t*, const float*, const float*, uint8_t*, int, int, int, int, hipStream_t);

template <class T>
int freq_mean(const T* P, float* out, long rows, int Fp, int C, hipStream_t st) {
  hipLaunchKernelGGL(freq_mean_kernel<T>, dim3(ew_grid(rows * C)), dim3(256), 0, st, P, out, rows, Fp, C);
  ACVAE_LAUNCH_CHECK();
  return ACVAE_OK;
}
template <class T>
int freq_mean_bwd(const float* dae, T* dP, long rows, int Fp, int C, hipStream_t st) {
  hipLaunchKernelGGL(freq_mean_bwd_kernel<T>, dim3(ew_grid(rows * Fp * C)), dim3(256), 0, st, dae, dP, rows, Fp, C);
  ACVAE_LAUNCH_CHECK();
  return ACVAE_OK;
}
template int freq_mean<float>(const float*, float*, long, int, int, hipStream_t);
template int freq_mean<bf16_t>(const bf16_t*, float*, long, int, int, hipStream_t);
template int freq_mean_bwd<float>(const float*, float*, long, int, int, hipStream_t);
template int freq_mean_bwd<bf16_t>(const float*, bf16_t*, long, int, int, hipStream_t);
int time_pool(const float* ae, float* out, int N, int S, int C, DropoutSpec drop, hipStream_t st) {
  hipLaunchKernelGGL(time_pool_kernel, dim3(ew_grid((long)N * C)), dim3(256), 0, st, ae, out, N, S, C, drop);
  ACVAE_LAUNCH_CHECK();
  return ACVAE_OK;
}
int relu_dropout(float* x, int total, DropoutSpec drop, hipStream_t st) {
  hipLaunchKernelGGL(relu_dropout_kernel, dim3(ew_grid(total)), dim3(256), 0, st, x, total, drop);
  ACVAE_LAUNCH_CHECK();
  return ACVAE_OK;
}

}
```

### acvae_amd/csrc/encoder.hip

```cpp
#include <algorithm>
#include "common.h"
#include "conv.h"
#include "resnet.h"
#include "../../include/acvae_hip.h"

namespace {

constexpr int kMaxBlocks = 6;
constexpr int kArchMask = 0xff;
constexpr int kChan[kMaxBlocks + 1] = {1, 64, 128, 256, 512, 1024, 2048};
struct Arch { int blocks; bool pool_last; };
inline bool arch_of(int arch, Arch& a) {
  if (arch & ~(kArchMask | ACVAE_ENC_BF16)) return false;
  if ((arch & kArchMask) == ACVAE_ARCH_CNN10) { a = {4, true}; return true; }
  if ((arch & kArchMask) == ACVAE_ARCH_CNN14_16K) { a = {6, false}; return true; }
  return false;
}
inline bool is_bf16(int arch) { return (arch & ACVAE_ENC_BF16) != 0; }
inline bool wino_on() {
  static const bool on = !getenv("ACVAE_CONV_WINO") || atoi(getenv("ACVAE_CONV_WINO")) != 0;
  return on;
}
template <class TA>
inline bool use_wino(int H, int W, int Cin, int Cout) {
// ... 421 lines not shown
  double* dpart = (double*)(scratch + L.s_dpart);
  const bool tr = training != 0;
  const float p_in = 0.5f * p_block;
  const DropoutSpec none{0.f, nullptr, 0, 0};
  auto dimg = [&](const R38Conv& c) { return tr ? saved + c.wd : wd; };
  ACVAE_TRY(acvae::colsum_tickets_reset(dpart, st));
  const int S = L.Hq, Wq = L.Wq;
  ACVAE_TRY(acvae::freq_mean_bwd<float>(d_audio_embeds, dyb, (long)N * S, Wq, 2048, st));
  const BnPtrs a1 = bn4(saved, L.a_bn1, 2048), a2 = bn4(saved, L.a_bn2, 2048);
  const int A = R38_AFTER;
  ACVAE_TRY(acvae::bn_bwd<float>(saved + L.a_y2, dyb, UP_DROP, a2.scale, a2.shift, a2.mean, a2.invstd, bnpart, G(A + 8), G(A + 7),
                                 dya, dpart, N, S, Wq, 2048, dspec(p_block, masks, seed, 18, training), st, tr));
  ACVAE_TRY(conv_wgrad<float>(dya, saved + L.a_y1, a1.scale, a1.shift, G(A + 1), slab, N, S, Wq, 2048, 2048, st));
  int red_rows = 0;
  acvae::WinoBnReduce red{saved + L.a_y1, a1.scale, a1.shift, a1.mean, a1.invstd};
  ACVAE_TRY(conv_dgrad<float>(dya, P(A + 1), dimg(L.a2), dyb, N, S, Wq, 2048, 2048, st, tr, &red, bnpart, &red_rows));
  ACVAE_TRY(acvae::bn_bwd<float>(saved + L.a_y1, dyb, UP_PLAIN, a1.scale, a1.shift, a1.mean, a1.invstd, bnpart, G(A + 3), G(A + 2),
                                 dya, dpart, N, S, Wq, 2048, none, st, tr, red_rows));
  ACVAE_TRY(conv_wgrad<float>(dya, saved + L.q, nullptr, nullptr, G(A), slab, N, S, Wq, 512, 2048, st));
  ACVAE_TRY(conv_dgrad<float>(dya, P(A), dimg(L.a1), dyb, N, S, Wq, 512, 2048, st, tr));
  if (block_done) ((void (*)(int, void*))block_done)(0, user);
  const R38Block& last = L.blk[R38_NB - 1];
  ACVAE_TRY(acvae::avg_pool2_bwd(dyb, nullptr, dcur, N, last.H, last.W, 512, 1, dspec(p_block, masks, seed, 17, training), st));
  for (int k = R38_NB - 1; k >= 0; --k) {
    const R38Block& B = L.blk[k];
    const long M = (long)N * B.H * B.W;
    const BnPtrs n1 = bn4(saved, B.bn1, B.C), n2 = bn4(saved, B.bn2, B.C);
    const BnPtrs nd = B.ds ? bn4(saved, B.bnd, B.C) : BnPtrs{nullptr, nullptr, nullptr, nullptr};
    const float* yd = B.ds ? saved + B.yd : nullptr;
    const int rows = acvae::res_join_rows(M, B.C);
    ACVAE_TRY(acvae::res_join_bwd_reduce(dcur, saved + B.out, saved + B.y2, n2.mean, n2.invstd, yd, nd.mean, nd.invstd, gbuf,
                                         bnpart, partd, M, B.C, st));
    ACVAE_TRY(acvae::colsum2(bnpart, rows, 2 * B.C, dpart, G(r38_p_bn2(B, 1)), G(r38_p_bn2(B, 0)), B.C, st));
    if (B.ds) ACVAE_TRY(acvae::colsum2(partd, rows, 2 * B.C, dpart, G(r38_p_dsbn(B, 1)), G(r38_p_dsbn(B, 0)), B.C, st));
    ACVAE_TRY(acvae::res_join_bwd_apply(gbuf, saved + B.y2, n2.scale, n2.mean, n2.invstd, G(r38_p_bn2(B, 1)), G(r38_p_bn2(B, 0)),
                                        dya, yd, nd.scale, nd.mean, nd.invstd, B.ds ? G(r38_p_dsbn(B, 1)) : nullptr,
                                        B.ds ? G(r38_p_dsbn(B, 0)) : nullptr, B.ds ? dyd : nullptr, M, B.C,
                                        tr ? 1.0f / (float)M : 0.f, st));
    ACVAE_TRY(conv_wgrad<float>(dya, saved + B.h1, nullptr, nullptr, G(r38_p_conv2(B)), slab, N, B.H, B.W, B.C, B.C, st));
    ACVAE_TRY(conv_dgrad<float>(dya, P(r38_p_conv2(B)), dimg(B.c2), dyb, N, B.H, B.W, B.C, B.C, st, tr));
    ACVAE_TRY(acvae::bn_bwd<float>(saved + B.y1, dyb, UP_DROP, n1.scale, n1.shift, n1.mean, n1.invstd, bnpart, G(r38_p_bn1(B, 1)),
                                   G(r38_p_bn1(B, 0)), dya, dpart, N, B.H, B.W, B.C, dspec(p_in, masks, seed, 1 + k, training),
                                   st, tr));
    const float* X = B.ds ? saved + B.xp : (k == 0 ? saved + L.x0 : saved + L.blk[k - 1].out);
    ACVAE_TRY(conv_wgrad<float>(dya, X, nullptr, nullptr, G(r38_p_conv1(B)), slab, N, B.H, B.W, B.Cin, B.C, st));
    ACVAE_TRY(conv_dgrad<float>(dya, P(r38_p_conv1(B)), dimg(B.c1), dxp, N, B.H, B.W, B.Cin, B.C, st, tr));
    if (B.ds) {
      ACVAE_TRY(acvae::conv1x1_wgrad(dyd, X, G(r38_p_dsw(B)), slab, M, B.Cin, B.C, st));
      ACVAE_TRY(acvae::conv1x1_dgrad(dyd, P(r38_p_dsw(B)), dxp, M, B.Cin, B.C, 1, st));
      ACVAE_TRY(acvae::avg_pool2_bwd(dxp, nullptr, dcur, N, B.Hin, B.Win, B.Cin, 1, none, st));
    } else {
      ACVAE_TRY(acvae::avg_pool2_bwd(dxp, gbuf, dcur, N, B.H, B.W, B.C, 0, none, st));
    }
  }
  const BnPtrs b0 = bn4(saved, L.bn0, 64), c1n1 = bn4(saved, L.c1_bn1, 64), c1n2 = bn4(saved, L.c1_bn2, 64);
  ACVAE_TRY(acvae::bn_bwd<float>(saved + L.c1_y2, dcur, UP_POOL, c1n2.scale, c1n2.shift, c1n2.mean, c1n2.invstd, bnpart, G(13),
                                 G(12), dya, dpart, N, T, F, 64, dspec(p_block, masks, seed, 0, training), st, tr));
  ACVAE_TRY(conv_wgrad<float>(dya, saved + L.c1_y1, c1n1.scale, c1n1.shift, G(6), slab, N, T, F, 64, 64, st));
  acvae::WinoBnReduce red1{saved + L.c1_y1, c1n1.scale, c1n1.shift, c1n1.mean, c1n1.invstd};
  ACVAE_TRY(conv_dgrad<float>(dya, P(6), dimg(L.cb1), dyb, N, T, F, 64, 64, st, tr, &red1, bnpart, &red_rows));
  ACVAE_TRY(acvae::bn_bwd<float>(saved + L.c1_y1, dyb, UP_PLAIN, c1n1.scale, c1n1.shift, c1n1.mean, c1n1.invstd, bnpart, G(8),
                                 G(7), dya, dpart, N, T, F, 64, none, st, tr, red_rows));
  ACVAE_TRY(acvae::conv1_first_bwd<float>(feats, b0.scale, b0.shift, b0.mean, b0.invstd, P(5), dya, scratch + L.s_c1w,
                                          scratch + L.s_c1b, G(5), G(0), G(1), dpart, N, T, F, st));
  return ACVAE_OK;
}

int r38_relu_mask(const void* saved_v, int64_t saved_bytes, int arch, int N, int T, int F, int site, uint8_t* mask,
                  hipStream_t st) {
  R38Layout L;
  ACVAE_TRY(make_r38_layout(arch, N, T, F, L));
  if (!saved_v || !mask || site < 0 || site >= 36) return ACVAE_EINVAL;
  if (saved_bytes < L.total * (int64_t)sizeof(float)) return ACVAE_EWORKSPACE;
  float* saved = (float*)saved_v;
  if (site < 2) {
    const BnPtrs b = bn4(saved, site ? L.c1_bn2 : L.c1_bn1, 64);
    return acvae::relu_mask<float>(saved + (site ? L.c1_y2 : L.c1_y1), b.scale, b.shift, mask, N, T, F, 64, st);
  }
  if (site >= 34) {
    const BnPtrs b = bn4(saved, site == 35 ? L.a_bn2 : L.a_bn1, 2048);
    return acvae::relu_mask<float>(saved + (site == 35 ? L.a_y2 : L.a_y1), b.scale, b.shift, mask, N, L.Hq, L.Wq, 2048, st);
  }
  const R38Block& B = L.blk[(site - 2) / 2];
  if (site % 2 == 0) {
    const BnPtrs b = bn4(saved, B.bn1, B.C);
    return acvae::relu_mask<float>(saved + B.y1, b.scale, b.shift, mask, N, B.H, B.W, B.C, st);
  }
  return acvae::positive_mask(saved + B.out, mask, N, B.H, B.W, B.C, st);
}
inline bool is_r38(int arch) { return (arch & kArchMask) == ACVAE_ARCH_RESNET38; }
}

extern "C" int acvae_encoder_nparams(int arch) {
  if (arch == ACVAE_ARCH_RESNET38) return R38_NPARAMS;
  Arch A;
  return arch_of(arch, A) ? 7 + A.blocks * 12 : -1;
}
extern "C" int acvae_encoder_out_dims(int arch, int T, int* S, int* C) {
  if (is_r38(arch)) {
    if (arch != ACVAE_ARCH_RESNET38 || T < 32 || !S || !C) return ACVAE_EINVAL;
    *S = T / 32;
    *C = 2048;
    return ACVAE_OK;
  }
  Arch A;
  if (!arch_of(arch, A) || !S || !C) return ACVAE_EINVAL;
  *S = T >> (A.pool_last ? A.blocks : A.blocks - 1);
  *C = kChan[A.blocks];
  return ACVAE_OK;
}
extern "C" int64_t acvae_encoder_saved_bytes(int arch, int N, int T, int F) {
  if (is_r38(arch)) {
    R38Layout R;
    return make_r38_layout(arch, N, T, F, R) == ACVAE_OK ? R.total * (int64_t)sizeof(float) : -1;
  }
  EncLayout L;
  if (make_layout(arch, N, T, F, L) != ACVAE_OK) return -1;
  return L.total * (int64_t)sizeof(float);
}
extern "C" int64_t acvae_encoder_scratch_bytes(int arch, int N, int T, int F) {
  if (is_r38(arch)) {
    R38Layout R;
    return make_r38_layout(arch, N, T, F, R) == ACVAE_OK ? R.s_total * (int64_t)sizeof(float) : -1;
  }
  EncLayout L;
  if (make_layout(arch, N, T, F, L) != ACVAE_OK) return -1;
  return L.s_total * (int64_t)sizeof(float);
}

namespace {
template <class TA>
int encoder_fwd_t(const void* const* params, const float* feats, float* audio_embeds, float* pooled,
                                 void* saved_v, int64_t saved_bytes, void* scratch_v, int64_t scratch_bytes, int arch,
                                 int N, int T, int F, int training, float p_block, float p_fc, uint64_t seed,
                                 const uint8_t* const* masks, void* stream) {
  EncLayout L;
  ACVAE_TRY(make_layout(arch, N, T, F, L));
  if (!params || !feats || !audio_embeds || !pooled || !saved_v || !scratch_v) return ACVAE_EINVAL;
  if (saved_bytes < L.total * (int64_t)sizeof(float) || scratch_bytes < L.s_total * (int64_t)sizeof(float))
    return ACVAE_EWORKSPACE;
  if (!aligned16(saved_v) || !aligned16(scratch_v) || !aligned16(feats)) return ACVAE_EALIGN;
  hipStream_t st = (hipStream_t)stream;
  float* saved = (float*)saved_v;
  float* scratch = (float*)scratch_v;
  float* partials = scratch + L.s_partials;
  double* dpart = (double*)(scratch + L.s_dpart);
  auto P = [&](int i) { return (float*)params[i]; };

  BnPtrs b0 = bn_at(saved, L, 0);
  int nparts = 0;
  ACVAE_TRY(acvae::colsum_tickets_reset(dpart, st));
  if (training) ACVAE_TRY(acvae::bn0_stats(feats, partials, (long)N * T, F, &nparts, st));
  ACVAE_TRY(acvae::bn_finalize(partials, nparts, 64, (double)N * T, P(p_bn0(0)), P(p_bn0(1)), P(p_bn0(2)), P(p_bn0(3)),
                               (int64_t*)params[p_bn0(4)], training, b0.scale, b0.shift, b0.mean, b0.invstd, dpart, st));
  bool wready[kMaxBlocks + 1][2] = {};
  if constexpr (sizeof(TA) == 4) {
    acvae::WinoWeightsBatch wb;
    for (int b = 1; b <= L.nb; ++b) {
      const int H = L.H[b], W = L.W[b], C = kChan[b], Cin = kChan[b - 1];
      if (b > 1 && use_wino<TA>(H, W, Cin, C)) {
        wb.add({P(p_conv(b, 1)), saved + L.wf1[b], C, Cin, false});
        if (training && use_wino<TA>(H, W, C, Cin)) wb.add({P(p_conv(b, 1)), saved + L.wd1[b], C, Cin, true});
        wready[b][0] = true;
      }
      if (use_wino<TA>(H, W, C, C)) {
        wb.add({P(p_conv(b, 2)), saved + L.wf2[b], C, C, false});
        if (training) wb.add({P(p_conv(b, 2)), saved + L.wd2[b], C, C, true});
        wready[b][1] = true;
      }
    }
    ACVAE_TRY(acvae::conv3x3_wino_weights_batch(wb, st));
  }
  {
    acvae::RepackBatch rb;
    for (int b = 1; b <= L.nb; ++b) {
      const int C = kChan[b], Cin = kChan[b - 1];
      if (b > 1 && !wready[b][0]) {
        rb.add({P(p_conv(b, 1)), saved + L.wf1[b], C, Cin, false});
        if (training) rb.add({P(p_conv(b, 1)), saved + L.wd1[b], C, Cin, true});
        wready[b][0] = true;
      }
      if (!wready[b][1]) {
        rb.add({P(p_conv(b, 2)), saved + L.wf2[b], C, C, false});
        if (training) rb.add({P(p_conv(b, 2)), saved + L.wd2[b], C, C, true});
        wready[b][1] = true;
      }
    }
    ACVAE_TRY(acvae::repack_weights_batch<TA>(rb, st));
  }
  const TA* x_in = nullptr;
  for (int b = 1; b <= L.nb; ++b) {
    const int H = L.H[b], W = L.W[b], C = kChan[b], Cin = kChan[b - 1];
    const double cnt = (double)N * H * W;
    TA* Y1 = (TA*)(saved + L.y1[b]);
    TA* Y2 = (TA*)(saved + L.y2[b]);
    BnPtrs n1 = bn_at(saved, L, 1 + 2 * (b - 1)), n2 = bn_at(saved, L, 2 + 2 * (b - 1));
    int np1;
    if (b == 1) {
      ACVAE_TRY(acvae::conv1_first_fwd(feats, b0.scale, b0.shift, P(p_conv(1, 1)), Y1, training ? partials : nullptr,
                                       N, T, F, st));
      np1 = acvae::conv1_first_blocks(N, T);
    } else {
      ACVAE_TRY(conv_fwd<TA>(x_in, nullptr, nullptr, P(p_conv(b, 1)), saved + L.wf1[b], Y1, training ? partials : nullptr, N,
                             H, W, Cin, C, &np1, st, wready[b][0]));
    }
    ACVAE_TRY(acvae::bn_finalize(partials, np1, C, cnt, P(p_bn(b, 1, 0)), P(p_bn(b, 1, 1)), P(p_bn(b, 1, 2)),
                                 P(p_bn(b, 1, 3)), (int64_t*)params[p_bn(b, 1, 4)], training, n1.scale, n1.shift,
                                 n1.mean, n1.invstd, dpart, st));
    int np2;
    ACVAE_TRY(conv_fwd<TA>((const TA*)Y1, n1.scale, n1.shift, P(p_conv(b, 2)), saved + L.wf2[b], Y2,
                           training ? partials : nullptr, N, H, W, C, C, &np2, st, wready[b][1]));
    ACVAE_TRY(acvae::bn_finalize(partials, np2, C, cnt, P(p_bn(b, 2, 0)),
                                 P(p_bn(b, 2, 1)), P(p_bn(b, 2, 2)), P(p_bn(b, 2, 3)), (int64_t*)params[p_bn(b, 2, 4)],
                                 training, n2.scale, n2.shift, n2.mean, n2.invstd, dpart, st));
    ACVAE_TRY(acvae::bn_relu_pool<TA>(Y2, n2.scale, n2.shift, (TA*)(saved + L.p[b]), N, H, W, C,
                                      dspec(p_block, masks, seed, b - 1, training), st, L.pool[b]));
    x_in = (const TA*)(saved + L.p[b]);
  }
  const int S = L.H[0], Fp = L.W[0], Ce = L.Cemb;
  ACVAE_TRY(acvae::freq_mean<TA>((const TA*)(saved + L.p[L.nb]), audio_embeds, (long)N * S, Fp, Ce, st));
  float* pin = saved + L.pooled_in;
  ACVAE_TRY(acvae::time_pool(audio_embeds, pin, N, S, Ce, dspec(p_fc, masks, seed, L.nb, training), st));
  ACVAE_TRY(acvae_gemm_nt_dual(pin, Ce, P(p_fc_w(L.nb)), Ce, Ce, nullptr, 0, nullptr, 0, 0, P(p_fc_b(L.nb)), pooled, Ce,
                               N, Ce, 0, st));
  ACVAE_TRY(acvae::relu_dropout(pooled, N * Ce, dspec(p_fc, masks, seed, L.nb + 1, training), st));
  return ACVAE_OK;
}
}

extern "C" int acvae_encoder_fwd(const void* const* params, const float* feats, float* audio_embeds, float* pooled,
                                 void* saved_v, int64_t saved_bytes, void* scratch_v, int64_t scratch_bytes, int arch,
                                 int N, int T, int F, int training, float p_block, float p_fc, uint64_t seed,
                                 const uint8_t* const* masks, void* stream) {
  if (is_r38(arch))
    return r38_fwd(params, feats, audio_embeds, pooled, saved_v, saved_bytes, scratch_v, scratch_bytes, arch, N, T, F, training,
                   p_block, p_fc, seed, masks, (hipStream_t)stream);
  if (is_bf16(arch))
    return encoder_fwd_t<bf16_t>(params, feats, audio_embeds, pooled, saved_v, saved_bytes, scratch_v, scratch_bytes, arch,
                                 N, T, F, training, p_block, p_fc, seed, masks, stream);
  return encoder_fwd_t<float>(params, feats, audio_embeds, pooled, saved_v, saved_bytes, scratch_v, scratch_bytes, arch, N,
                              T, F, training, p_block, p_fc, seed, masks, stream);
}

extern "C" int acvae_encoder_relu_mask(const void* saved_v, int64_t saved_bytes, int arch, int N, int T, int F, int site,
                                       uint8_t* mask_nchw, void* stream) {
  if (is_r38(arch)) return r38_relu_mask(saved_v, saved_bytes, arch, N, T, F, site, mask_nchw, (hipStream_t)stream);
  EncLayout L;
  ACVAE_TRY(make_layout(arch, N, T, F, L));
  if (!saved_v || !mask_nchw || site < 0 || site >= 2 * L.nb) return ACVAE_EINVAL;
  if (saved_bytes < L.total * (int64_t)sizeof(float)) return ACVAE_EWORKSPACE;
  float* saved = (float*)saved_v;
  const int b = site / 2 + 1, which = site % 2;
  BnPtrs bn = bn_at(saved, L, 1 + 2 * (b - 1) + which);
  const long off = which ? L.y2[b] : L.y1[b];
  if (is_bf16(arch))
    return acvae::relu_mask<bf16_t>((const bf16_t*)(saved + off), bn.scale, bn.shift, mask_nchw, N, L.H[b], L.W[b], kChan[b],
                                    (hipStream_t)stream);
  return acvae::relu_mask<float>(saved + off, bn.scale, bn.shift, mask_nchw, N, L.H[b], L.W[b], kChan[b], (hipStream_t)stream);
}

namespace {
template <class TA>
int encoder_bwd_t(const void* const* params, void* const* grads, const float* feats,
                                 const float* d_audio_embeds, void* saved_v, int64_t saved_bytes, void* scratch_v,
                                 int64_t scratch_bytes, int arch, int N, int T, int F, int training, float p_block,
                                 uint64_t seed, const uint8_t* const* masks, void* stream, void* block_done,
                                 void* user) {
  EncLayout L;
  ACVAE_TRY(make_layout(arch, N, T, F, L));
  if (!params || !grads || !feats || !d_audio_embeds || !saved_v || !scratch_v) return ACVAE_EINVAL;
  if (saved_bytes < L.total * (int64_t)sizeof(float) || scratch_bytes < L.s_total * (int64_t)sizeof(float))
    return ACVAE_EWORKSPACE;
  hipStream_t st = (hipStream_t)stream;
  float* saved = (float*)saved_v;
  float* scratch = (float*)scratch_v;
  auto P = [&](int i) { return (float*)params[i]; };
  auto G = [&](int i) { return (float*)grads[i]; };
  TA* dya = (TA*)(scratch + L.s_dya);
  TA* dyb = (TA*)(scratch + L.s_dyb);
  TA* dp_cur = (TA*)(scratch + L.s_dpa);
  TA* dp_nxt = (TA*)(scratch + L.s_dpb);
  TA* wd = (TA*)(scratch + L.s_wd);
  float* slab = scratch + L.s_slab;
  float* bnpart = scratch + L.s_bnpart;
  double* dpart = (double*)(scratch + L.s_dpart);
  const int S = L.H[0], Fp = L.W[0];
  ACVAE_TRY(acvae::colsum_tickets_reset(dpart, st));
  ACVAE_TRY(acvae::freq_mean_bwd<TA>(d_audio_embeds, dp_cur, (long)N * S, Fp, L.Cemb, st));
  for (int b = L.nb; b >= 1; --b) {
    const int H = L.H[b], W = L.W[b], C = kChan[b], Cin = kChan[b - 1];
    const TA* Y1 = (const TA*)(saved + L.y1[b]);
    const TA* Y2 = (const TA*)(saved + L.y2[b]);
    BnPtrs n1 = bn_at(saved, L, 1 + 2 * (b - 1)), n2 = bn_at(saved, L, 2 + 2 * (b - 1));
    ACVAE_TRY(acvae::bn_bwd<TA>(Y2, dp_cur, L.pool[b] ? UP_POOL : UP_DROP, n2.scale, n2.shift, n2.mean, n2.invstd, bnpart, G(p_bn(b, 2, 1)),
                            G(p_bn(b, 2, 0)), dya, dpart, N, H, W, C, dspec(p_block, masks, seed, b - 1, training), st,
                            training != 0));
    ACVAE_TRY(conv_wgrad<TA>((const TA*)dya, Y1, n1.scale, n1.shift, G(p_conv(b, 2)), slab, N, H, W, C, C, st));
    const bool wd_ready = training != 0;
    int red_rows = 0;
    acvae::WinoBnReduce red{(const float*)Y1, n1.scale, n1.shift, n1.mean, n1.invstd};
    ACVAE_TRY(conv_dgrad<TA>((const TA*)dya, P(p_conv(b, 2)), wd_ready ? (TA*)(saved + L.wd2[b]) : wd, dyb, N, H, W, C, C, st, wd_ready,
                             sizeof(TA) == 4 ? &red : nullptr, bnpart, &red_rows));
    DropoutSpec none{0.f, nullptr, 0, 0};
    ACVAE_TRY(acvae::bn_bwd<TA>(Y1, dyb, UP_PLAIN, n1.scale, n1.shift, n1.mean, n1.invstd, bnpart, G(p_bn(b, 1, 1)),
                            G(p_bn(b, 1, 0)), dya, dpart, N, H, W, C, none, st, training != 0, red_rows));
    if (b > 1) {
      ACVAE_TRY(conv_wgrad<TA>((const TA*)dya, (const TA*)(saved + L.p[b - 1]), nullptr, nullptr, G(p_conv(b, 1)), slab, N, H,
                               W, Cin, C, st));
      const bool fw = use_wino<TA>(H, W, Cin, C), dw = use_wino<TA>(H, W, C, Cin);
      const bool r1 = wd_ready && fw == dw;
      ACVAE_TRY(conv_dgrad<TA>((const TA*)dya, P(p_conv(b, 1)), r1 ? (TA*)(saved + L.wd1[b]) : wd, dp_nxt, N, H, W, Cin, C, st, r1));
      TA* t = dp_cur; dp_cur = dp_nxt; dp_nxt = t;
    } else {
      BnPtrs b0 = bn_at(saved, L, 0);
      ACVAE_TRY(acvae::conv1_first_bwd<TA>(feats, b0.scale, b0.shift, b0.mean, b0.invstd, P(p_conv(1, 1)), (const TA*)dya,
                                       scratch + L.s_c1w, scratch + L.s_c1b, G(p_conv(1, 1)), G(p_bn0(0)), G(p_bn0(1)),
                                       dpart, N, T, F, st));
    }
    if (block_done) ((void (*)(int, void*))block_done)(b, user);
  }
  return ACVAE_OK;
}
}

extern "C" int acvae_encoder_bwd_hooked(const void* const* params, void* const* grads, const float* feats,
                                 const float* d_audio_embeds, void* saved_v, int64_t saved_bytes, void* scratch_v,
                                 int64_t scratch_bytes, int arch, int N, int T, int F, int training, float p_block,
                                 uint64_t seed, const uint8_t* const* masks, void* stream, void* block_done,
                                 void* user) {
  if (is_r38(arch))
    return r38_bwd(params, grads, feats, d_audio_embeds, saved_v, saved_bytes, scratch_v, scratch_bytes, arch, N, T, F, training,
                   p_block, seed, masks, (hipStream_t)stream, block_done, user);
  if (is_bf16(arch))
    return encoder_bwd_t<bf16_t>(params, grads, feats, d_audio_embeds, saved_v, saved_bytes, scratch_v, scratch_bytes, arch,
                                 N, T, F, training, p_block, seed, masks, stream, block_done, user);
  return encoder_bwd_t<float>(params, grads, feats, d_audio_embeds, saved_v, saved_bytes, scratch_v, scratch_bytes, arch, N,
                              T, F, training, p_block, seed, masks, stream, block_done, user);
}

extern "C" int acvae_encoder_bwd(const void* const* params, void* const* grads, const float* feats,
                                 const float* d_audio_embeds, void* saved_v, int64_t saved_bytes, void* scratch_v,
                                 int64_t scratch_bytes, int arch, int N, int T, int F, int training, float p_block,
                                 uint64_t seed, const uint8_t* const* masks, void* stream) {
  return acvae_encoder_bwd_hooked(params, grads, feats, d_audio_embeds, saved_v, saved_bytes, scratch_v, scratch_bytes,
                                  arch, N, T, F, training, p_block, seed, masks, stream, nullptr, nullptr);
}
```

### acvae_amd/csrc/ops_abi.hip

```cpp
#include "common.h"
#include "conv.h"
#include "rnn.h"
#include "../../include/acvae_hip.h"

namespace {
inline long al64(long x) { return (x + 63) & ~63L; }

struct ConvWs {
  long wp, partials, dpart, slab, total;
};
ConvWs conv_ws(int N, int H, int W, int Cin, int Cout) {
  ConvWs w;
  long o = 0;
  w.wp = o; o = al64(o + (long)Cout * 16 * Cin);
  long part = Cin == 1 ? (long)acvae::conv1_first_blocks(N, H) * 128 : (long)acvae::conv_partials_rows(N, H, W) * 2 * Cout;
  if (Cin > 1 && W >= 4 && W % 2 == 0 && (long)acvae::conv_wino_partials_rows(N, H, W) * 2 * Cout > part)
    part = (long)acvae::conv_wino_partials_rows(N, H, W) * 2 * Cout;
  w.partials = o; o = al64(o + part);
  w.dpart = o; o = al64(o + 2 * acvae::colsum_scratch_doubles(2 * Cout > 1024 ? 2 * Cout : 1024));
  long slab = Cin == 1 ? (long)acvae::conv1_first_blocks(N, H) * (576 + 128)
                       : acvae::conv3x3_wgrad_slab_floats(N, H, W, Cin, Cout);
  if (Cin % 64 == 0) {
    const long sb = acvae::conv3x3_wgrad_bf16_slab_floats(N, H, W, Cin, Cout);
    if (sb > slab) slab = sb;
  }
  if (Cin > 1) {
    const long sw = acvae::conv3x3_wino_wgrad_slab_floats(N, H, W, Cin, Cout);
    if (sw > slab) slab = sw;
  }
  w.slab = o; o = al64(o + slab);
  w.total = o;
  return w;
}
bool conv_dims_ok(int N, int H, int W, int Cin, int Cout) {
  return N > 0 && H > 0 && W > 0 && Cin > 0 && Cout > 0 && (long)N * H * W < (1L << 31);
}
}

extern "C" int64_t acvae_conv3x3_workspace_bytes(int N, int H, int W, int Cin, int Cout) {
  if (!conv_dims_ok(N, H, W, Cin, Cout)) return -1;
  return conv_ws(N, H, W, Cin, Cout).total * 4;
}

extern "C" int acvae_conv3x3_fwd(const float* X, const float* W_oihw, const float* in_scale, const float* in_shift,
                                 float* Y, const float* gamma, const float* beta, float* running_mean,
                                 float* running_var, int64_t* num_batches_tracked, int training, float* bn_out,
                                 void* ws_v, int64_t ws_bytes, int N, int H, int W, int Cin, int Cout, void* stream) {
  if (!conv_dims_ok(N, H, W, Cin, Cout) || !X || !W_oihw || !Y || !ws_v) return ACVAE_EINVAL;
  if ((in_scale == nullptr) != (in_shift == nullptr)) return ACVAE_EINVAL;
  if (bn_out && (!gamma || !beta || !running_mean || !running_var)) return ACVAE_EINVAL;
  const ConvWs L = conv_ws(N, H, W, Cin, Cout);
  if (ws_bytes < L.total * 4) return ACVAE_EWORKSPACE;
  if (!aligned16(ws_v)) return ACVAE_EALIGN;
  hipStream_t st = (hipStream_t)stream;
  float* ws = (float*)ws_v;
  float* partials = (bn_out && training) ? ws + L.partials : nullptr;
  int nparts;
  if (Cin == 1) {
    if (W != 64 || Cout != 64 || !in_scale) return ACVAE_EUNSUPPORTED;
    ACVAE_TRY(acvae::conv1_first_fwd(X, in_scale, in_shift, W_oihw, Y, partials, N, H, W, st));
    nparts = acvae::conv1_first_blocks(N, H);
  } else {
    ACVAE_TRY(acvae::repack_weights<float>(W_oihw, ws + L.wp, nullptr, Cout, Cin, st));
    ACVAE_TRY(acvae::conv3x3_igemm(X, in_scale, in_shift, ws + L.wp, Y, partials, N, H, W, Cin, Cout, st));
    nparts = acvae::conv_partials_rows(N, H, W);
  }
  if (bn_out) ACVAE_TRY(acvae::colsum_tickets_reset((double*)(ws + L.dpart), st));
  if (bn_out)
    ACVAE_TRY(acvae::bn_finalize(partials, nparts, Cout, (double)N * H * W, gamma, beta, running_mean, running_var,
                                 num_batches_tracked, training, bn_out, bn_out + Cout, bn_out + 2 * Cout,
                                 bn_out + 3 * Cout, (double*)(ws + L.dpart), st));
  return ACVAE_OK;
}

extern "C" int acvae_conv3x3_dgrad(const float* dY, const float* W_oihw, float* dX, void* ws_v, int64_t ws_bytes, int N,
                                   int H, int W, int Cin, int Cout, void* stream) {
  if (!conv_dims_ok(N, H, W, Cin, Cout) || !dY || !W_oihw || !dX || !ws_v) return ACVAE_EINVAL;
  if (Cin == 1) return ACVAE_EUNSUPPORTED;
  const ConvWs L = conv_ws(N, H, W, Cin, Cout);
  if (ws_bytes < L.total * 4) return ACVAE_EWORKSPACE;
  hipStream_t st = (hipStream_t)stream;
  float* ws = (float*)ws_v;
  ACVAE_TRY(acvae::repack_weights<float>(W_oihw, nullptr, ws + L.wp, Cout, Cin, st));
  return acvae::conv3x3_igemm(dY, nullptr, nullptr, ws + L.wp, dX, nullptr, N, H, W, Cout, Cin, st);
}

extern "C" int acvae_conv3x3_wgrad(const float* dY, const float* X, const float* in_scale, const float* in_shift,
                                   float* dW_oihw, void* ws_v, int64_t ws_bytes, int N, int H, int W, int Cin, int Cout,
                                   void* stream) {
  if (!conv_dims_ok(N, H, W, Cin, Cout) || !dY || !X || !dW_oihw || !ws_v) return ACVAE_EINVAL;
  if ((in_scale == nullptr) != (in_shift == nullptr)) return ACVAE_EINVAL;
  if (Cin == 1) return ACVAE_EUNSUPPORTED;
  const ConvWs L = conv_ws(N, H, W, Cin, Cout);
  if (ws_bytes < L.total * 4) return ACVAE_EWORKSPACE;
  return acvae::conv3x3_wgrad(dY, X, in_scale, in_shift, dW_oihw, (float*)ws_v + L.slab, N, H, W, Cin, Cout,
                              (hipStream_t)stream);
}

extern "C" int acvae_conv3x3_fwd_wino(const float* X, const float* W_oihw, const float* in_scale, const float* in_shift,
                                      float* Y, const float* gamma, const float* beta, float* running_mean,
                                      float* running_var, int64_t* num_batches_tracked, int training, float* bn_out,
                                      void* ws_v, int64_t ws_bytes, int N, int H, int W, int Cin, int Cout, void* stream) {
  if (!conv_dims_ok(N, H, W, Cin, Cout) || !X || !W_oihw || !Y || !ws_v) return ACVAE_EINVAL;
  if ((in_scale == nullptr) != (in_shift == nullptr)) return ACVAE_EINVAL;
  if (bn_out && (!gamma || !beta || !running_mean || !running_var)) return ACVAE_EINVAL;
  if (!acvae::conv3x3_wino_ok(H, W, Cin, Cout)) return ACVAE_EUNSUPPORTED;
  const ConvWs L = conv_ws(N, H, W, Cin, Cout);
  if (ws_bytes < L.total * 4) return ACVAE_EWORKSPACE;
  if (!aligned16(ws_v)) return ACVAE_EALIGN;
  hipStream_t st = (hipStream_t)stream;
  float* ws = (float*)ws_v;
  float* partials = (bn_out && training) ? ws + L.partials : nullptr;
  ACVAE_TRY(acvae::conv3x3_wino_weights(W_oihw, ws + L.wp, Cout, Cin, false, st));
  ACVAE_TRY(acvae::conv3x3_wino(X, in_scale, in_shift, ws + L.wp, Y, partials, N, H, W, Cin, Cout, st));
  if (bn_out) ACVAE_TRY(acvae::colsum_tickets_reset((double*)(ws + L.dpart), st));
  if (bn_out)
    ACVAE_TRY(acvae::bn_finalize(partials, acvae::conv_wino_partials_rows(N, H, W), Cout, (double)N * H * W, gamma, beta,
                                 running_mean, running_var, num_batches_tracked, training, bn_out, bn_out + Cout,
                                 bn_out + 2 * Cout, bn_out + 3 * Cout, (double*)(ws + L.dpart), st));
  return ACVAE_OK;
}

extern "C" int acvae_conv3x3_dgrad_wino(const float* dY, const float* W_oihw, float* dX, void* ws_v, int64_t ws_bytes, int N,
                                        int H, int W, int Cin, int Cout, void* stream) {
  if (!conv_dims_ok(N, H, W, Cin, Cout) || !dY || !W_oihw || !dX || !ws_v) return ACVAE_EINVAL;
  if (!acvae::conv3x3_wino_ok(H, W, Cout, Cin)) return ACVAE_EUNSUPPORTED;
  const ConvWs L = conv_ws(N, H, W, Cin, Cout);
  if (ws_bytes < L.total * 4) return ACVAE_EWORKSPACE;
  if (!aligned16(ws_v)) return ACVAE_EALIGN;
  hipStream_t st = (hipStream_t)stream;
  float* ws = (float*)ws_v;
  ACVAE_TRY(acvae::conv3x3_wino_weights(W_oihw, ws + L.wp, Cout, Cin, true, st));
  return acvae::conv3x3_wino(dY, nullptr, nullptr, ws + L.wp, dX, nullptr, N, H, W, Cout, Cin, st);
}

extern "C" int acvae_conv3x3_dgrad_bnred_wino(const float* dY, const float* W_oihw, float* dX, const float* Yprev, const float* bn_prev,
                                              float* sum_g, float* sum_gy, void* ws_v, int64_t ws_bytes, int N, int H, int W, int Cin,
                                              int Cout, void* stream) {
  if (!conv_dims_ok(N, H, W, Cin, Cout) || !dY || !W_oihw || !dX || !Yprev || !bn_prev || !sum_g || !sum_gy || !ws_v) return ACVAE_EINVAL;
  if (!acvae::conv3x3_wino_ok(H, W, Cout, Cin)) return ACVAE_EUNSUPPORTED;
  const ConvWs L = conv_ws(N, H, W, Cin, Cout);
  const ConvWs Lr = conv_ws(N, H, W, Cout, Cin);
  if (ws_bytes < L.total * 4 || ws_bytes < Lr.total * 4) return ACVAE_EWORKSPACE;
  if (!aligned16(ws_v)) return ACVAE_EALIGN;
  hipStream_t st = (hipStream_t)stream;
  float* ws = (float*)ws_v;
  ACVAE_TRY(acvae::colsum_tickets_reset((double*)(ws + Lr.dpart), st));
  ACVAE_TRY(acvae::conv3x3_wino_weights(W_oihw, ws + L.wp, Cout, Cin, true, st));
  const acvae::WinoBnReduce red{Yprev, bn_prev, bn_prev + Cin, bn_prev + 2 * Cin, bn_prev + 3 * Cin};
  ACVAE_TRY(acvae::conv3x3_wino(dY, nullptr, nullptr, ws + L.wp, dX, ws + Lr.partials, N, H, W, Cout, Cin, st, &red));
  return acvae::colsum2(ws + Lr.partials, acvae::conv_wino_partials_rows(N, H, W), 2 * Cin, (double*)(ws + Lr.dpart), sum_g, sum_gy, Cin, st);
}

extern "C" int acvae_conv3x3_wgrad_wino(const float* dY, const float* X, const float* in_scale, const float* in_shift,
                                        float* dW_oihw, void* ws_v, int64_t ws_bytes, int N, int H, int W, int Cin, int Cout,
                                        void* stream) {
  if (!conv_dims_ok(N, H, W, Cin, Cout) || !dY || !X || !dW_oihw || !ws_v) return ACVAE_EINVAL;
  if ((in_scale == nullptr) != (in_shift == nullptr)) return ACVAE_EINVAL;
  if (!acvae::conv3x3_wino_wgrad_ok(H, W, Cin, Cout)) return ACVAE_EUNSUPPORTED;
  const ConvWs L = conv_ws(N, H, W, Cin, Cout);
  if (ws_bytes < L.total * 4) return ACVAE_EWORKSPACE;
  if (!aligned16(ws_v)) return ACVAE_EALIGN;
  return acvae::conv3x3_wino_wgrad(dY, X, in_scale, in_shift, dW_oihw, (float*)ws_v + L.slab, N, H, W, Cin, Cout,
                                   (hipStream_t)stream);
}

extern "C" int acvae_conv3x3_fwd_bf16(const void* X, const float* W_oihw, const float* in_scale, const float* in_shift,
                                      void* Y, const float* gamma, const float* beta, float* running_mean,
                                      float* running_var, int64_t* num_batches_tracked, int training, float* bn_out,
                                      void* ws_v, int64_t ws_bytes, int N, int H, int W, int Cin, int Cout, void* stream) {
  if (!conv_dims_ok(N, H, W, Cin, Cout) || !X || !W_oihw || !Y || !ws_v) return ACVAE_EINVAL;
  if ((in_scale == nullptr) != (in_shift == nullptr)) return ACVAE_EINVAL;
  if (bn_out && (!gamma || !beta || !running_mean || !running_var)) return ACVAE_EINVAL;
  if (Cin % 64 != 0) return ACVAE_EUNSUPPORTED;
  const ConvWs L = conv_ws(N, H, W, Cin, Cout);
  if (ws_bytes < L.total * 4) return ACVAE_EWORKSPACE;
  if (!aligned16(ws_v)) return ACVAE_EALIGN;
  hipStream_t st = (hipStream_t)stream;
  float* ws = (float*)ws_v;
  float* partials = (bn_out && training) ? ws + L.partials : nullptr;
  bf16_t* wp = (bf16_t*)(ws + L.wp);
  ACVAE_TRY(acvae::repack_weights<bf16_t>(W_oihw, wp, nullptr, Cout, Cin, st));
  ACVAE_TRY(acvae::conv3x3_igemm_bf16((const bf16_t*)X, in_scale, in_shift, wp, (bf16_t*)Y, partials, N, H, W, Cin, Cout, st));
  if (bn_out) ACVAE_TRY(acvae::colsum_tickets_reset((double*)(ws + L.dpart), st));
  if (bn_out)
    ACVAE_TRY(acvae::bn_finalize(partials, acvae::conv_partials_rows(N, H, W), Cout, (double)N * H * W, gamma, beta,
                                 running_mean, running_var, num_batches_tracked, training, bn_out, bn_out + Cout,
                                 bn_out + 2 * Cout, bn_out + 3 * Cout, (double*)(ws + L.dpart), st));
  return ACVAE_OK;
}

extern "C" int acvae_conv3x3_dgrad_bf16(const void* dY, const float* W_oihw, void* dX, void* ws_v, int64_t ws_bytes, int N,
                                        int H, int W, int Cin, int Cout, void* stream) {
  if (!conv_dims_ok(N, H, W, Cin, Cout) || !dY || !W_oihw || !dX || !ws_v) return ACVAE_EINVAL;
  if (Cin % 64 != 0 || Cout % 64 != 0) return ACVAE_EUNSUPPORTED;
  const ConvWs L = conv_ws(N, H, W, Cin, Cout);
  if (ws_bytes < L.total * 4) return ACVAE_EWORKSPACE;
  hipStream_t st = (hipStream_t)stream;
  bf16_t* wd = (bf16_t*)((float*)ws_v + L.wp);
  ACVAE_TRY(acvae::repack_weights<bf16_t>(W_oihw, nullptr, wd, Cout, Cin, st));
  return acvae::conv3x3_igemm_bf16((const bf16_t*)dY, nullptr, nullptr, wd, (bf16_t*)dX, nullptr, N, H, W, Cout, Cin, st);
}

extern "C" int acvae_conv3x3_wgrad_bf16(const void* dY, const void* X, const float* in_scale, const float* in_shift,
                                        float* dW_oihw, void* ws_v, int64_t ws_bytes, int N, int H, int W, int Cin,
                                        int Cout, void* stream) {
  if (!conv_dims_ok(N, H, W, Cin, Cout) || !dY || !X || !dW_oihw || !ws_v) return ACVAE_EINVAL;
  if ((in_scale == nullptr) != (in_shift == nullptr)) return ACVAE_EINVAL;
  if (Cin % 64 != 0) return ACVAE_EUNSUPPORTED;
  const ConvWs L = conv_ws(N, H, W, Cin, Cout);
  if (ws_bytes < L.total * 4) return ACVAE_EWORKSPACE;
  return acvae::conv3x3_wgrad((const bf16_t*)dY, (const bf16_t*)X, in_scale, in_shift, dW_oihw, (float*)ws_v + L.slab, N, H,
                              W, Cin, Cout, (hipStream_t)stream);
}

extern "C" int acvae_conv1_first_bwd(const float* x, const float* bn0, const float* W1_oihw, const float* dY, float* dW1,
                                     float* dgamma0, float* dbeta0, void* ws_v, int64_t ws_bytes, int N, int T, int F,
                                     void* stream) {
  if (N <= 0 || T <= 0 || !x || !bn0 || !W1_oihw || !dY || !dW1 || !dgamma0 || !dbeta0 || !ws_v) return ACVAE_EINVAL;
  if (F != 64) return ACVAE_EUNSUPPORTED;
  const ConvWs L = conv_ws(N, T, F, 1, 64);
  if (ws_bytes < L.total * 4) return ACVAE_EWORKSPACE;
  float* ws = (float*)ws_v;
  const long nb = acvae::conv1_first_blocks(N, T);
  ACVAE_TRY(acvae::colsum_tickets_reset((double*)(ws + L.dpart), (hipStream_t)stream));
  return acvae::conv1_first_bwd(x, bn0, bn0 + 64, bn0 + 128, bn0 + 192, W1_oihw, dY, ws + L.slab, ws + L.slab + nb * 576,
                                dW1, dgamma0, dbeta0, (double*)(ws + L.dpart), N, T, F, (hipStream_t)stream);
}

extern "C" int64_t acvae_bn_workspace_bytes(int N, int H, int W, int C) {
  if (N <= 0 || H <= 0 || W <= 0 || C <= 0) return -1;
  const long part = (long)acvae::bn_bwd_blocks(N, H, W, C) * 2 * C;
  const long p0 = (long)acvae::bn0_partials_rows((long)N * H) * 128;
  return (al64(part > p0 ? part : p0) + al64(2 * acvae::colsum_scratch_doubles(2 * C > 1024 ? 2 * C : 1024))) * 4;
}

extern "C" int acvae_bn_mel_fwd(const float* x, const float* gamma, const float* beta, float* running_mean,
                                float* running_var, int64_t* num_batches_tracked, int training, float* bn_out,
                                void* ws_v, int64_t ws_bytes, int64_t rows, int F, void* stream) {
  if (rows <= 0 || !x || !gamma || !beta || !running_mean || !running_var || !bn_out || !ws_v) return ACVAE_EINVAL;
  if (F != 64) return ACVAE_EUNSUPPORTED;
  const long part = al64((long)acvae::bn0_partials_rows(rows) * 128);
  if (ws_bytes < (part + al64(2 * acvae::colsum_scratch_doubles(1024))) * 4) return ACVAE_EWORKSPACE;
  hipStream_t st = (hipStream_t)stream;
  float* ws = (float*)ws_v;
  int nparts = 0;
  if (training) ACVAE_TRY(acvae::bn0_stats(x, ws, rows, F, &nparts, st));
  ACVAE_TRY(acvae::colsum_tickets_reset((double*)(ws + part), st));
  return acvae::bn_finalize(ws, nparts, F, (double)rows, gamma, beta, running_mean, running_var, num_batches_tracked,
                            training, bn_out, bn_out + F, bn_out + 2 * F, bn_out + 3 * F, (double*)(ws + part), st);
}

extern "C" int acvae_bn_relu_pool_fwd(const float* Y, const float* bn, float* P, int N, int H, int W, int C, int pool,
                                      float p_drop, uint64_t seed, int site, const uint8_t* keep_mask, void* stream) {
  if (N <= 0 || H <= 0 || W <= 0 || C <= 0 || !Y || !bn || !P) return ACVAE_EINVAL;
  DropoutSpec d{p_drop, keep_mask, seed, (uint32_t)site};
  return acvae::bn_relu_pool(Y, bn, bn + C, P, N, H, W, C, d, (hipStream_t)stream, pool != 0);
}

extern "C" int acvae_bn_relu_bwd(const float* Y, const float* dO, int upstream, const float* bn, float* dgamma,
                                 float* dbeta, float* dY, void* ws_v, int64_t ws_bytes, int N, int H, int W, int C,
                                 int training, float p_drop, uint64_t seed, int site, const uint8_t* keep_mask,
                                 void* stream) {
  if (N <= 0 || H <= 0 || W <= 0 || C <= 0 || !Y || !dO || !bn || !dgamma || !dbeta || !dY || !ws_v) return ACVAE_EINVAL;
  if (upstream != UP_PLAIN && upstream != UP_POOL && upstream != UP_DROP) return ACVAE_EINVAL;
  if (ws_bytes < acvae_bn_workspace_bytes(N, H, W, C)) return ACVAE_EWORKSPACE;
  float* ws = (float*)ws_v;
  const long part = al64((long)acvae::bn_bwd_blocks(N, H, W, C) * 2 * C);
  const long p0 = al64((long)acvae::bn0_partials_rows((long)N * H) * 128);
  DropoutSpec d{p_drop, keep_mask, seed, (uint32_t)site};
  ACVAE_TRY(acvae::colsum_tickets_reset((double*)(ws + (part > p0 ? part : p0)), (hipStream_t)stream));
  return acvae::bn_bwd(Y, dO, upstream, bn, bn + C, bn + 2 * C, bn + 3 * C, ws, dbeta, dgamma, dY,
                       (double*)(ws + (part > p0 ? part : p0)), N, H, W, C, d, (hipStream_t)stream, training != 0);
}

extern "C" int64_t acvae_rnn_workspace_bytes(int N, int Tc, int I, int H) {
  if (N <= 0 || Tc <= 0 || I <= 0 || H <= 0) return -1;
  const long R = (long)N * Tc;
  return (al64(acvae_skinny_ws_floats()) + al64(R * 8 * H) + al64((long)N * 4 * H) + al64((long)N * H) +
          al64(R * 5 * H) + al64(R * H)) * 4;
}

extern "C" int acvae_gru_step(const float* x, const float* h, const float* w_ih, const float* w_hh, const float* b_ih,
                              const float* b_hh, float* h_out, void* ws_v, int64_t ws_bytes, int N, int I, int H,
                              void* stream) {
  if (N <= 0 || I <= 0 || H <= 0 || !x || !h || !w_ih || !w_hh || !h_out || !ws_v) return ACVAE_EINVAL;
  if (ws_bytes < acvae_rnn_workspace_bytes(N, 1, I, H)) return ACVAE_EWORKSPACE;
  hipStream_t st = (hipStream_t)stream;
  float* ws = (float*)ws_v;
  float* sk = ws;
  float* gi = ws + al64(acvae_skinny_ws_floats());
  float* gh = gi + al64((long)N * 8 * H);
  ACVAE_TRY(acvae_skinny_ws_reset(sk, st));
  ACVAE_TRY(acvae_gemm_nt_dual(x, I, w_ih, I, I, nullptr, 0, nullptr, 0, 0, b_ih, gi, 3 * H, N, 3 * H, 0, st, sk));
  ACVAE_TRY(acvae_gemm_nt_dual(h, H, w_hh, H, H, nullptr, 0, nullptr, 0, 0, b_hh, gh, 3 * H, N, 3 * H, 0, st, sk));
  return acvae::gru_fwd(gi, 3 * H, gh, 3 * H, h, H, h_out, H, nullptr, 0, nullptr, 0, nullptr, 0, nullptr, 0, N, H, st);
}

extern "C" int acvae_lstm_step(const float* x, const float* h, const float* c, const float* w_ih, const float* w_hh,
                               const float* b_ih, const float* b_hh, float* h_out, float* c_out, void* ws_v,
                               int64_t ws_bytes, int N, int I, int H, void* stream) {
  if (N <= 0 || I <= 0 || H <= 0 || !x || !h || !c || !w_ih || !w_hh || !h_out || !c_out || !ws_v) return ACVAE_EINVAL;
  if (ws_bytes < acvae_rnn_workspace_bytes(N, 1, I, H)) return ACVAE_EWORKSPACE;
  hipStream_t st = (hipStream_t)stream;
  float* ws = (float*)ws_v;
  float* sk = ws;
  float* gates = ws + al64(acvae_skinny_ws_floats());
  ACVAE_TRY(acvae_skinny_ws_reset(sk, st));
  ACVAE_TRY(acvae_gemm_nt_dual(x, I, w_ih, I, I, nullptr, 0, nullptr, 0, 0, b_ih, gates, 4 * H, N, 4 * H, 0, st, sk));
  ACVAE_TRY(acvae_gemm_nt_dual(h, H, w_hh, H, H, nullptr, 0, nullptr, 0, 0, b_hh, gates, 4 * H, N, 4 * H, 1, st, sk));
  return acvae::lstm_fwd(gates, 4 * H, c, H, h_out, H, c_out, H, nullptr, 0, N, H, st);
}

extern "C" int acvae_bigru_seq(const float* X, const int64_t* lens, const void* const* w, float* hidden, void* ws_v,
                               int64_t ws_bytes, int N, int Tc, int E, int H, void* stream) {
  if (N <= 0 || Tc <= 0 || E <= 0 || H <= 0 || !X || !lens || !w || !hidden || !ws_v) return ACVAE_EINVAL;
  for (int i = 0; i < 8; ++i)
    if (!w[i]) return ACVAE_EINVAL;
  if (ws_bytes < acvae_rnn_workspace_bytes(N, Tc, E, H)) return ACVAE_EWORKSPACE;
  hipStream_t st = (hipStream_t)stream;
  const long R = (long)N * Tc;
  float* ws = (float*)ws_v;
  float* sk = ws;
  float* gi = ws + al64(acvae_skinny_ws_floats());
  float* gh = gi + al64(R * 8 * H);
  float* hcur = gh + al64((long)N * 4 * H);
  float* save = hcur + al64((long)N * H);
  float* hps = save + al64(R * 5 * H);
  ACVAE_TRY(acvae_skinny_ws_reset(sk, st));
  for (int dir = 0; dir < 2; ++dir) {
    const float* wih = (const float*)w[dir * 4 + 0];
    const float* whh = (const float*)w[dir * 4 + 1];
    const float* bih = (const float*)w[dir * 4 + 2];
    const float* bhh = (const float*)w[dir * 4 + 3];
    ACVAE_TRY(acvae_gemm_nt_dual(X, E, wih, E, E, nullptr, 0, nullptr, 0, 0, bih, gi, 3 * H, (int)R, 3 * H, 0, st, sk));
    ACVAE_TRY(acvae::copy_rows(hcur, H, nullptr, 0, N, H, st));
    for (int k = 0; k < Tc; ++k) {
      const int t = dir ? Tc - 1 - k : k;
      ACVAE_TRY(acvae_gemm_nt_dual(hcur, H, whh, H, H, nullptr, 0, nullptr, 0, 0, bhh, gh, 3 * H, N, 3 * H, 0, st, sk));
      ACVAE_TRY(acvae::gru_fwd(gi + (long)t * 3 * H, (long)Tc * 3 * H, gh, 3 * H, hcur, H, hcur, H,
                               hidden + (long)t * 2 * H + dir * H, (long)Tc * 2 * H, save + (long)t * 4 * H,
                               (long)Tc * 4 * H, hps + (long)t * H, (long)Tc * H, lens, t, N, H, st));
    }
  }
  return ACVAE_OK;
}

extern "C" int64_t acvae_colsum_workspace_bytes(int cols) {
  return cols > 0 ? al64(2 * acvae::colsum_scratch_doubles(cols)) * 4 : -1;
}
extern "C" int acvae_colsum(const float* x, int rows, int cols, float* out, void* ws, int64_t ws_bytes, void* stream) {
  if (!x || !out || !ws || rows <= 0 || cols <= 0) return ACVAE_EINVAL;
  if (ws_bytes < acvae_colsum_workspace_bytes(cols)) return ACVAE_EWORKSPACE;
  ACVAE_TRY(acvae::colsum_tickets_reset((double*)ws, (hipStream_t)stream));
  return acvae::colsum2(x, rows, cols, (double*)ws, out, nullptr, 0, (hipStream_t)stream);
}

static int colsum_table(int n, const int* P, const int* width, acvae::ColsumBatch& b) {
  if (n <= 0 || n > acvae::ColsumBatch::capacity || !P || !width) return ACVAE_EINVAL;
  for (int j = 0; j < n; ++j) {
    if (P[j] <= 0 || width[j] <= 0) return ACVAE_EINVAL;
    b.add({nullptr, P[j], width[j], nullptr, nullptr, 0, 0});
  }
  return ACVAE_OK;
}
extern "C" int64_t acvae_colsum_batch_workspace_bytes(int n, const int* P, const int* width) {
  acvae::ColsumBatch b;
  if (colsum_table(n, P, width, b) != ACVAE_OK) return -1;
  long d = 0;
  acvae::colsum_batch_plan(b, 0, &d);
  return ((int64_t)acvae::colsum_ticket_words() / 2 + d) * 8;
}
extern "C" int acvae_colsum_batch_plan(int n, const int* P, const int* width, int64_t ws_bytes) {
  acvae::ColsumBatch b;
  ACVAE_TRY(colsum_table(n, P, width, b));
  return acvae::colsum_batch_plan(b, (long)(ws_bytes / 8), nullptr) ? 1 : 0;
}
extern "C" int acvae_colsum_batch(int n, const void* const* x, const int* P, const int* width, const void* const* out,
                                  const void* const* out_b, void* ws, int64_t ws_bytes, int reset_tickets, void* stream) {
  acvae::ColsumBatch b;
  ACVAE_TRY(colsum_table(n, P, width, b));
  if (!x || !out || !ws) return ACVAE_EINVAL;
  for (int j = 0; j < n; ++j) {
    if (!x[j] || !out[j]) return ACVAE_EINVAL;
    b.job[j].x = (const float*)x[j];
    b.job[j].out = (float*)out[j];
    b.job[j].out_b = out_b ? (float*)out_b[j] : nullptr;
  }
  acvae::ColsumBatch plan = b;
  acvae::colsum_batch_plan(plan, 0, nullptr);
  for (int j = 0; j < n; ++j)
    if (ws_bytes < ((int64_t)acvae::colsum_ticket_words() / 2 + (int64_t)plan.job[j].R * width[j]) * 8) return ACVAE_EWORKSPACE;
  hipStream_t st = (hipStream_t)stream;
  if (reset_tickets) ACVAE_TRY(acvae::colsum_tickets_reset((double*)ws, st));
  return acvae::colsum_batch(b, (double*)ws, (long)(ws_bytes / 8), st);
}
```

### include/acvae_hip.h

```cpp
#ifndef ACVAE_HIP_H
#define ACVAE_HIP_H
#include <stdint.h>
#ifdef __cplusplus
extern "C" {
#endif

#define ACVAE_ABI_VERSION 3
int acvae_abi_version(void);

#define ACVAE_FLAG_NO_PERSIST 1
#define ACVAE_FLAG_DEFER_PARAM_GRADS 2
#define ACVAE_FLAG_NO_ATTN_SPLIT 4
#define ACVAE_FLAG_TEST_STALL 8

int acvae_persist_status_register(int device, void* status_words_host);

int acvae_gemm_nt(const float* A, int64_t lda, const float* B, int64_t ldb, const float* bias, float* C,
                  int64_t ldc, int M, int N, int K, int accumulate, void* stream);
int acvae_gemm_tn(const float* A, int64_t lda, const float* B, int64_t ldb, float* C, int64_t ldc, int M, int N,
                  int K, int accumulate, float* slab_ws, int64_t slab_ws_bytes, void* stream);
int64_t acvae_gemm_tn_workspace_bytes(int M, int N, int K);
int64_t acvae_colsum_workspace_bytes(int cols);
int acvae_colsum(const float* x, int rows, int cols, float* out, void* ws, int64_t ws_bytes, void* stream);

int64_t acvae_gemm_nt_splitk_workspace_bytes(void);
int acvae_gemm_nt_split_plan(int M, int N, int K1, int K2, int with_ws);
int acvae_gemm_nt_dual_ws(const float* A1, int64_t lda1, const float* B1, int64_t ldb1, int K1, const float* A2,
                          int64_t lda2, const float* B2, int64_t ldb2, int K2, const float* bias, float* C, int64_t ldc,
                          int M, int N, int accumulate, float* ws, int64_t ws_bytes, int reset_tickets, void* stream);
int acvae_gemm_nt_pair_c(const float* A0, int64_t lda0, const float* B0, int64_t ldb0, int K0, const float* bias0, float* C0,
                         int64_t ldc0, int N0, int acc0, const float* A1, int64_t lda1, const float* B1, int64_t ldb1, int K1,
                         const float* bias1, float* C1, int64_t ldc1, int N1, int acc1, int M, void* stream);
int64_t acvae_gemm_tn_fused_workspace_bytes(int M, int N, int K);
int acvae_gemm_tn_fused_plan(int M, int N, int K, int64_t ws_bytes);
int acvae_gemm_tn_fused_c(const float* A, int64_t lda, const float* B, int64_t ldb, float* C, int64_t ldc, int M, int N,
                          int K, int accumulate, float* ws, int64_t ws_bytes, int reset_tickets, void* stream);
int64_t acvae_colsum_batch_workspace_bytes(int n, const int* P, const int* width);
int acvae_colsum_batch_plan(int n, const int* P, const int* width, int64_t ws_bytes);
int acvae_colsum_batch(int n, const void* const* x, const int* P, const int* width, const void* const* out,
                       const void* const* out_b, void* ws, int64_t ws_bytes, int reset_tickets, void* stream);
int acvae_transpose(const float* in, int64_t ld_in, float* out, int64_t ld_out, int rows, int cols, void* stream);

int64_t acvae_attn_fwd_workspace_bytes(int N, int Tq, int S, int A, int E);
int acvae_attn_fwd(const float* qproj, int64_t q_sn, int64_t q_sj, const float* encproj, const float* enc,
                   const int64_t* lens, const float* v, float* ctx, int64_t c_sn, int64_t c_sj, float* weights,
                   int64_t w_sn, int64_t w_sj, int N, int Tq, int S, int A, int E, void* ws, int64_t ws_bytes, void* stream,
                   int flags);
int acvae_tanh_att(const float* x, float* y, int64_t n, void* stream);
int64_t acvae_attn_bwd_workspace_bytes(int N, int Tq, int S, int A);
int acvae_attn_bwd(const float* dctx, int64_t dc_sn, int64_t dc_sj, const float* qproj, int64_t q_sn, int64_t q_sj,
                   const float* encproj, const float* enc, const int64_t* lens, const float* v,
                   const float* weights, int64_t w_sn, int64_t w_sj, float* dqproj, int64_t dq_sn, int64_t dq_sj,
                   float* dencproj, float* denc, float* dv_part, float* ws, int64_t ws_bytes, int N, int Tq, int S,
                   int A, int E, void* stream);

int acvae_reparam_fwd(const float* ml, int64_t ld_ml, const float* eps, int64_t ld_eps, float* mean, float* logv,
                      float* z, int64_t ld_out, float* z2, int64_t ld_z2, int rows, int E, void* stream);
int acvae_reparam_bwd(const float* dz, int64_t ld_dz, const float* dmean_ext, const float* dlog_ext, int64_t ld_ext,
                      const float* logv, int64_t ld_lv, const float* eps, int64_t ld_eps, float* dml, int64_t ld_dml,
                      int rows, int E, void* stream);

int64_t acvae_kl_partials(int64_t n_elem);
int acvae_gauss_kl_fwd(const float* mu1, const float* lv1, const float* mu2, const float* lv2, float* partials,
                       float* out_scalar, int64_t rows, int E, void* stream);
int acvae_gauss_kl_bwd(const float* mu1, const float* lv1, const float* mu2, const float* lv2, const float* grad_out,
                       float* dmu1, float* dlv1, float* dmu2, float* dlv2, int64_t rows, int E, void* stream);

int acvae_row_logsoftmax_argmax(const float* logits, int64_t ld_n, int64_t ld_t, int64_t* argmax, float* max_logprob,
                                float* lse, int64_t o_sn, int64_t o_st, int N, int T, int V, void* stream);
#define ACVAE_SAMPLE_GREEDY 0
#define ACVAE_SAMPLE_GUMBEL 1
#define ACVAE_SAMPLE_MULTINOMIAL 2
int acvae_sample_noise(float* noise, int64_t n, int method, uint64_t seed, void* stream);
int acvae_sample_next_word(const float* logits, int64_t ld_n, int64_t ld_t, const float* noise, int64_t nz_sn,
                           int64_t nz_st, int method, float temp, int64_t* w_out, float* logprob_out, int64_t o_sn,
                           int64_t o_st, int N, int T, int V, void* stream);
int acvae_ls_ce_fwd(const float* logits, int64_t ld_n, int64_t ld_t, const int64_t* targets, int64_t tg_sn,
                    const int64_t* lens1, const float* lse, float smoothing, int reduction, float* loss_rows,
                    float* out_scalar, int N, int T, int V, void* stream);
int acvae_ls_ce_bwd(const float* logits, int64_t ld_n, int64_t ld_t, const int64_t* targets, int64_t tg_sn,
                    const int64_t* lens1, const float* lse, float smoothing, int reduction, const float* grad_out,
                    const float* grad_rows, float* dlogits, int N, int T, int V, void* stream);
int acvae_mse_fwd(const float* a, const float* b, float* partials, float* out_scalar, int64_t n, void* stream);
int acvae_mse_bwd(const float* a, const float* b, const float* grad_out, float* da, float* db, int64_t n, void* stream);
int acvae_loss_combine_fwd(const float* ce, const float* kl, const float* mse, float w_kl, float w_mse, float* out, void* stream);
int acvae_loss_combine_bwd(const float* grad_out, float w_kl, float w_mse, float* g_ce, float* g_kl, float* g_mse, void* stream);

#define ACVAE_ENC_NPARAMS 55
#define ACVAE_ARCH_CNN10 0
#define ACVAE_ARCH_CNN14_16K 1
#define ACVAE_ARCH_RESNET38 2
#define ACVAE_ENC_BF16 256
int acvae_encoder_nparams(int arch);
int acvae_encoder_out_dims(int arch, int T, int* S, int* C);
int64_t acvae_encoder_saved_bytes(int arch, int N, int T, int F);
int64_t acvae_encoder_scratch_bytes(int arch, int N, int T, int F);
int acvae_encoder_fwd(const void* const* params, const float* feats, float* audio_embeds, float* pooled,
                      void* saved, int64_t saved_bytes, void* scratch, int64_t scratch_bytes, int arch, int N, int T,
                      int F, int training, float p_block, float p_fc, uint64_t seed, const uint8_t* const* masks,
                      void* stream);
int acvae_encoder_bwd(const void* const* params, void* const* grads, const float* feats,
                      const float* d_audio_embeds, void* saved, int64_t saved_bytes, void* scratch,
                      int64_t scratch_bytes, int arch, int N, int T, int F, int training, float p_block, uint64_t seed,
                      const uint8_t* const* masks, void* stream);
int acvae_encoder_relu_mask(const void* saved, int64_t saved_bytes, int arch, int N, int T, int F, int site,
                            uint8_t* mask_nchw, void* stream);
int acvae_encoder_bwd_hooked(const void* const* params, void* const* grads, const float* feats,
                             const float* d_audio_embeds, void* saved, int64_t saved_bytes, void* scratch,
                             int64_t scratch_bytes, int arch, int N, int T, int F, int training, float p_block,
                             uint64_t seed, const uint8_t* const* masks, void* stream, void* block_done, void* user);

int64_t acvae_conv3x3_workspace_bytes(int N, int H, int W, int Cin, int Cout);
int acvae_conv3x3_fwd(const float* X, const float* W_oihw, const float* in_scale, const float* in_shift, float* Y,
                      const float* gamma, const float* beta, float* running_mean, float* running_var,
                      int64_t* num_batches_tracked, int training, float* bn_out, void* ws, int64_t ws_bytes, int N, int H,
                      int W, int Cin, int Cout, void* stream);
int acvae_conv3x3_dgrad(const float* dY, const float* W_oihw, float* dX, void* ws, int64_t ws_bytes, int N, int H, int W,
                        int Cin, int Cout, void* stream);
int acvae_conv3x3_wgrad(const float* dY, const float* X, const float* in_scale, const float* in_shift, float* dW_oihw,
                        void* ws, int64_t ws_bytes, int N, int H, int W, int Cin, int Cout, void* stream);
int acvae_conv1_first_bwd(const float* x, const float* bn0, const float* W1_oihw, const float* dY, float* dW1,
                          float* dgamma0, float* dbeta0, void* ws, int64_t ws_bytes, int N, int T, int F, void* stream);
int acvae_conv3x3_fwd_wino(const float* X, const float* W_oihw, const float* in_scale, const float* in_shift, float* Y,
                           const float* gamma, const float* beta, float* running_mean, float* running_var,
                           int64_t* num_batches_tracked, int training, float* bn_out, void* ws, int64_t ws_bytes, int N,
                           int H, int W, int Cin, int Cout, void* stream);
int acvae_conv3x3_dgrad_wino(const float* dY, const float* W_oihw, float* dX, void* ws, int64_t ws_bytes, int N, int H,
                             int W, int Cin, int Cout, void* stream);
int acvae_conv3x3_dgrad_bnred_wino(const float* dY, const float* W_oihw, float* dX, const float* Yprev, const float* bn_prev,
                                   float* sum_g, float* sum_gy, void* ws, int64_t ws_bytes, int N, int H, int W, int Cin,
                                   int Cout, void* stream);
int acvae_conv3x3_wgrad_wino(const float* dY, const float* X, const float* in_scale, const float* in_shift, float* dW_oihw,
                             void* ws, int64_t ws_bytes, int N, int H, int W, int Cin, int Cout, void* stream);
int acvae_conv3x3_fwd_bf16(const void* X, const float* W_oihw, const float* in_scale, const float* in_shift, void* Y,
                           const float* gamma, const float* beta, float* running_mean, float* running_var,
                           int64_t* num_batches_tracked, int training, float* bn_out, void* ws, int64_t ws_bytes, int N,
                           int H, int W, int Cin, int Cout, void* stream);
int acvae_conv3x3_dgrad_bf16(const void* dY, const float* W_oihw, void* dX, void* ws, int64_t ws_bytes, int N, int H, int W,
                             int Cin, int Cout, void* stream);
int acvae_conv3x3_wgrad_bf16(const void* dY, const void* X, const float* in_scale, const float* in_shift, float* dW_oihw,
                             void* ws, int64_t ws_bytes, int N, int H, int W, int Cin, int Cout, void* stream);
int64_t acvae_bn_workspace_bytes(int N, int H, int W, int C);
int acvae_res_join_fwd(const float* y2, const float* bn2, const float* yd, const float* bnd, const float* x, float* out, int N,
                       int H, int W, int C, void* stream);
int64_t acvae_res_join_bwd_workspace_bytes(int N, int H, int W, int C);
int acvae_res_join_bwd(const float* dO, const float* out, const float* y2, const float* bn2, const float* yd, const float* bnd,
                       float* G, float* dy2, float* dyd, float* dgamma2, float* dbeta2, float* dgammad, float* dbetad,
                       int training, void* ws, int64_t ws_bytes, int N, int H, int W, int C, void* stream);
int acvae_conv1x1_partials_rows(int N, int H, int W);
int acvae_conv1x1_fwd(const float* X, const float* W_oi, float* Y, float* partials, int N, int H, int W, int Cin, int Cout,
                      void* stream);
int acvae_conv1x1_dgrad(const float* dY, const float* W_oi, float* dX, int accumulate, int N, int H, int W, int Cin, int Cout,
                        void* stream);
int64_t acvae_conv1x1_wgrad_workspace_bytes(int N, int H, int W, int Cin, int Cout);
int acvae_conv1x1_wgrad(const float* dY, const float* X, float* dW_oi, void* ws, int64_t ws_bytes, int N, int H, int W, int Cin,
                        int Cout, void* stream);
int acvae_avg_pool2_fwd(const float* X, float* P, int N, int H, int W, int C, float p_drop, uint64_t seed, int site,
                        const uint8_t* mask, void* stream);
int acvae_avg_pool2_bwd(const float* dP, const float* add, float* dX, int N, int H, int W, int C, int pool, float p_drop,
                        uint64_t seed, int site, const uint8_t* mask, void* stream);
int acvae_bn_mel_fwd(const float* x, const float* gamma, const float* beta, float* running_mean, float* running_var,
                     int64_t* num_batches_tracked, int training, float* bn_out, void* ws, int64_t ws_bytes, int64_t rows,
                     int F, void* stream);
int acvae_bn_relu_pool_fwd(const float* Y, const float* bn, float* P, int N, int H, int W, int C, int pool, float p_drop,
                           uint64_t seed, int site, const uint8_t* keep_mask, void* stream);
int acvae_bn_relu_bwd(const float* Y, const float* dO, int upstream, const float* bn, float* dgamma, float* dbeta,
                      float* dY, void* ws, int64_t ws_bytes, int N, int H, int W, int C, int training, float p_drop,
                      uint64_t seed, int site, const uint8_t* keep_mask, void* stream);

int64_t acvae_rnn_workspace_bytes(int N, int Tc, int I, int H);
int acvae_gru_step(const float* x, const float* h, const float* w_ih, const float* w_hh, const float* b_ih,
                   const float* b_hh, float* h_out, void* ws, int64_t ws_bytes, int N, int I, int H, void* stream);
int acvae_lstm_step(const float* x, const float* h, const float* c, const float* w_ih, const float* w_hh,
                    const float* b_ih, const float* b_hh, float* h_out, float* c_out, void* ws, int64_t ws_bytes, int N,
                    int I, int H, void* stream);
int acvae_bigru_seq(const float* X, const int64_t* lens, const void* const* w, float* hidden, void* ws, int64_t ws_bytes,
                    int N, int Tc, int E, int H, void* stream);

#define ACVAE_TEXT_NPARAMS 35

int64_t acvae_posterior_saved_bytes(int N, int Tc, int E, int Hq, int V);
int64_t acvae_posterior_scratch_bytes(int N, int Tc, int E, int Hq, int V);
int acvae_posterior_fwd(const void* const* params, const int64_t* caps, int64_t ld_caps, const int64_t* lens1,
                        const float* eps_q, float* q_means, float* q_logs, float* q_z, float* q_means_utt,
                        void* saved, int64_t saved_bytes, void* scratch, int64_t scratch_bytes, int N, int Tc, int E,
                        int Hq, int V, void* stream, int flags);
int acvae_posterior_bwd(const void* const* params, void* const* grads, const int64_t* lens1, const float* eps_q,
                        const float* q_logs, const float* d_q_means, const float* d_q_logs, const float* d_q_z,
                        const float* d_q_means_utt, void* saved, int64_t saved_bytes, void* scratch,
                        int64_t scratch_bytes, int N, int Tc, int E, int Hq, int V, void* stream, int flags);

int64_t acvae_posterior_stack_saved_bytes(int N, int Tc, int E, int Hq, int V, int num_layers);
int64_t acvae_posterior_stack_scratch_bytes(int N, int Tc, int E, int Hq, int V, int num_layers);
int acvae_posterior_stack_fwd(const void* const* params, const void* const* upper, int num_layers, const uint8_t* keep,
                              float keep_scale, const int64_t* caps, int64_t ld_caps, const int64_t* lens1,
                              const float* eps_q, float* q_means, float* q_logs, float* q_z, float* q_means_utt,
                              void* saved, int64_t saved_bytes, void* scratch, int64_t scratch_bytes, int N, int Tc,
                              int E, int Hq, int V, void* stream, int flags);
int acvae_posterior_stack_bwd(const void* const* params, void* const* grads, const void* const* upper,
                              void* const* upper_grads, int num_layers, const uint8_t* keep, float keep_scale,
                              const int64_t* lens1, const float* eps_q, const float* q_logs, const float* d_q_means,
                              const float* d_q_logs, const float* d_q_z, const float* d_q_means_utt, void* saved,
                              int64_t saved_bytes, void* scratch, int64_t scratch_bytes, int N, int Tc, int E, int Hq,
                              int V, void* stream, int flags);


int64_t acvae_decode_saved_bytes(int N, int Tc, int S, int E, int H, int A, int V, int Eenc);
int64_t acvae_decode_scratch_bytes(int N, int Tc, int S, int E, int H, int A, int V, int Eenc);
int acvae_decode_fwd(const void* const* params, const float* mem_in, const int64_t* mem_lens, const int64_t* caps,
                     int64_t ld_caps, const int64_t* lens1, const float* q_z, const float* eps_p,
                     const int* ss_flags_host, const int* dis_flags_host, float* logits, float* outputs, int64_t* seqs,
                     float* sampled_logprobs, float* attn_w, float* p_means, float* p_logs, float* p_z,
                     float* p_means_utt, float* h_final, float* hp_final, float* cp_final, void* saved,
                     int64_t saved_bytes, void* scratch, int64_t scratch_bytes, int N, int Tc, int S, int E, int H,
                     int A, int V, int Eenc, int start_idx, int end_idx, void* stream, void* aux_stream, int flags);
int acvae_decode_fwd_sampled(const void* const* params, const float* mem_in, const int64_t* mem_lens,
                             const int64_t* caps, int64_t ld_caps, const int64_t* lens1, const float* q_z,
                             const float* eps_p, const int* ss_flags_host, const int* dis_flags_host, float* logits,
                             float* outputs, int64_t* seqs, float* sampled_logprobs, float* attn_w, float* p_means,
                             float* p_logs, float* p_z, float* p_means_utt, float* h_final, float* hp_final,
                             float* cp_final, void* saved, int64_t saved_bytes, void* scratch, int64_t scratch_bytes,
                             int N, int Tc, int S, int E, int H, int A, int V, int Eenc, int start_idx, int end_idx,
                             void* stream, void* aux_stream, int sample_method, float temp, const float* sample_noise,
                             const uint8_t* emb_keep, float emb_drop_p, int flags);
int acvae_decode_bwd_defers(const int* dis_flags_host, int Tc, void* stream, void* aux_stream, int flags);
int acvae_decode_bwd(const void* const* params, void* const* grads, const float* mem_in, const int64_t* mem_lens,
                     const int64_t* lens1, const float* eps_p, const int* dis_flags_host, const float* outputs,
                     const float* attn_w, const float* p_logs, const float* d_logits, const float* d_outputs_ext,
                     const float* d_p_means, const float* d_p_logs, const float* d_p_z, const float* d_p_means_utt,
                     float* d_mem_in, float* d_q_z, void* saved, int64_t saved_bytes, void* scratch,
                     int64_t scratch_bytes, int N, int Tc, int S, int E, int H, int A, int V, int Eenc, void* stream,
                     void* aux_stream, const uint8_t* emb_keep, float emb_drop_p, int flags);
int acvae_caps_to_long(const float* caps, int64_t* out, int64_t n, void* stream);

int64_t acvae_grad_norm_partials(void);
int acvae_grad_norm(const float* grads, int64_t n, float grad_scale, float* partials, float* out_norm, void* stream);
int acvae_adam_step(float* params, const float* grads, float* exp_avg, float* exp_avg_sq, int64_t n, float lr,
                    float beta1, float beta2, float eps, float weight_decay, int64_t step, float grad_scale,
                    float max_grad_norm, const float* total_norm, void* stream);
int acvae_adamw_step(float* params, const float* grads, float* exp_avg, float* exp_avg_sq, float* max_exp_avg_sq,
                     int64_t n, double lr, double beta1, double beta2, double eps, double weight_decay, int decoupled,
                     int amsgrad, int64_t step, float grad_scale, float max_grad_norm, const float* total_norm,
                     void* stream);
int acvae_sgd_step(float* params, const float* grads, float* momentum_buffer, int64_t n, double lr, double momentum,
                   double dampening, double weight_decay, int nesterov, int first, float grad_scale, float max_grad_norm,
                   const float* total_norm, void* stream);

#define ACVAE_AUG_MAX_MASKS 8
#define ACVAE_AUG_TABLE_WIDTH 35
#define ACVAE_AUG_MAX_F 1024
int acvae_spec_augment(const float* in, float* out, const int* lens, const int* params, int N, int T, int F, int K,
                       void* stream);

int acvae_prof_enable(int enable);
int acvae_prof_pause(int paused);
int acvae_prof_read(int tag, double* total_ms_host, int64_t* launches_host);

int64_t acvae_step_scratch_bytes(int N, int S, int E, int H, int A, int V);
int acvae_attn_precompute(const void* const* params, int which, const float* mem, float* encproj, int N, int S, int E,
                          int H, int A, void* stream);
int acvae_prior_step_fwd(const void* const* params, const int64_t* word, const float* mem, const int64_t* mem_lens,
                         const float* encproj_p, const float* h_prev, const float* c_prev, const float* last_z,
                         const float* eps, float* mean, float* logv, float* z, float* h_out, float* c_out, float* attw,
                         void* scratch, int64_t scratch_bytes, int N, int S, int E, int V, void* stream);
int acvae_decoder_step_fwd(const void* const* params, const int64_t* word, const float* h_prev, const float* mem,
                           const int64_t* mem_lens, const float* encproj_d, const float* z, float* logits, float* h_out,
                           float* attw, float* rnn_input, void* scratch, int64_t scratch_bytes, int N, int S, int E,
                           int H, int A, int V, void* stream);
int acvae_logprob_add(const float* logits, int64_t ld, const float* lse, const float* prev, float* out, int N, int V,
                      void* stream);
int acvae_topk_flat(const float* x, int64_t n, int k, int V, float* vals, int64_t* idx, int64_t* row, int64_t* col,
                    void* stream);
int acvae_topk_flat_batched(const float* x, int64_t n, int64_t group_stride, int k, int V, float* vals, int64_t* idx,
                            int64_t* row, int64_t* col, int groups, int row_base, void* stream);
int64_t acvae_beam_search_scratch_bytes(int N, int beam, int max_length, int S, int E, int H, int A, int V);
int acvae_beam_search(const void* const* params, const float* mem, const int64_t* mem_lens, const float* eps,
                      int64_t start_idx, int64_t* seqs, float* attn_weights, void* scratch, int64_t scratch_bytes, int N,
                      int beam, int max_length, int S, int E, int H, int A, int V, void* stream);
int acvae_dbs_scores(const float* logits, int64_t ld, float temperature, const float* counts, float diversity_lambda,
                     const float* prev, float* out, int N, int V, int rows_per_count, void* stream);

#ifdef __cplusplus
}
#endif
#endif
```

Measured before the change: 2023.

## Fold first-block BatchNorm backward apply into conv1 weight-gradient kernel

For the first encoder block in fp32, the BatchNorm-backward elementwise apply pass is skipped; only the reduction sums run, and the conv1_first_bwd kernel recomputes the BN/ReLU gradient on the fly from Y1 and the upstream gradient while accumulating the weight gradient. This removes one full read-write pass over the largest activation tensor (64 channels at full resolution) and a kernel launch. In exchange the conv1 kernel loads two tensors per pixel, holds more registers (the launch bounds now request 3 blocks per SM), and needs a small shared table of per-channel constants. The BN math is also factored into a shared header.

```diff
diff --git a/acvae_amd/csrc/bn_bwd.h b/acvae_amd/csrc/bn_bwd.h
--- /dev/null
+++ b/acvae_amd/csrc/bn_bwd.h
@@ -0,0 +1,39 @@
+#pragma once
+#include <hip/hip_runtime.h>
+
+struct BnBwdQuad { float4 sc, sh, mu, is, a, b; };
+
+__device__ __forceinline__ BnBwdQuad bn_bwd_quad(const float* __restrict__ scale, const float* __restrict__ shift,
+                                                 const float* __restrict__ mean, const float* __restrict__ invstd,
+                                                 const float* __restrict__ sum_g, const float* __restrict__ sum_gy, int c,
+                                                 float invn) {
+  BnBwdQuad k;
+  k.sc = *reinterpret_cast<const float4*>(scale + c); k.sh = *reinterpret_cast<const float4*>(shift + c);
+  k.mu = *reinterpret_cast<const float4*>(mean + c); k.is = *reinterpret_cast<const float4*>(invstd + c);
+  k.a = *reinterpret_cast<const float4*>(sum_g + c); k.b = *reinterpret_cast<const float4*>(sum_gy + c);
+  k.a.x *= invn; k.a.y *= invn; k.a.z *= invn; k.a.w *= invn;
+  k.b.x *= invn; k.b.y *= invn; k.b.z *= invn; k.b.w *= invn;
+  return k;
+}
+
+__device__ __forceinline__ float bn_bwd_dz1(float y, float g, float sc, float sh, float mu, float is, float a, float b) {
+  if (y * sc + sh <= 0.f) g = 0.f;
+  return sc * (g - a - ((y - mu) * is) * b);
+}
+__device__ __forceinline__ float4 bn_bwd_dz(float4 y, float4 g, const BnBwdQuad& k) {
+  return make_float4(bn_bwd_dz1(y.x, g.x, k.sc.x, k.sh.x, k.mu.x, k.is.x, k.a.x, k.b.x),
+                     bn_bwd_dz1(y.y, g.y, k.sc.y, k.sh.y, k.mu.y, k.is.y, k.a.y, k.b.y),
+                     bn_bwd_dz1(y.z, g.z, k.sc.z, k.sh.z, k.mu.z, k.is.z, k.a.z, k.b.z),
+                     bn_bwd_dz1(y.w, g.w, k.sc.w, k.sh.w, k.mu.w, k.is.w, k.a.w, k.b.w));
+}
+
+__host__ __device__ inline float bn_bwd_invn(int N, int H, int W, bool batch_stats) {
+  return batch_stats ? 1.0f / (float)((long)N * H * W) : 0.f;
+}
+
+struct BnBwdApply {
+  const float* Y;
+  const float* scale; const float* shift; const float* mean; const float* invstd;
+  const float* sum_g; const float* sum_gy;
+  float invn;
+};
diff --git a/acvae_amd/csrc/conv.h b/acvae_amd/csrc/conv.h
--- a/acvae_amd/csrc/conv.h
+++ b/acvae_amd/csrc/conv.h
@@ -3,6 +3,7 @@
 #include <stdint.h>
 #include "common.h"
 #include "job_table.h"
+#include "bn_bwd.h"
 
 struct DropoutSpec {
   float p;
@@ -81,7 +82,7 @@
 template <class TY>
 int conv1_first_bwd(const float* x, const float* scale0, const float* shift0, const float* mean0, const float* invstd0,
                     const float* W1, const TY* dY, float* dw_part, float* bn_part, float* dW1, float* dgamma0,
-                    float* dbeta0, double* dpart, int N, int T, int F, hipStream_t st);
+                    float* dbeta0, double* dpart, int N, int T, int F, hipStream_t st, const BnBwdApply* bn = nullptr);
 template <class T>
 int bn_relu_pool(const T* Y, const float* scale, const float* shift, T* P, int N, int H, int W, int C,
                  DropoutSpec drop, hipStream_t st, bool pool = true);
@@ -90,6 +91,10 @@
 int bn_bwd(const T* Y, const T* dO, int upstream, const float* scale, const float* shift, const float* mean,
            const float* invstd, float* partials, float* sum_g, float* sum_gy, T* dY, double* dpart, int N, int H,
            int W, int C, DropoutSpec drop, hipStream_t st, bool batch_stats = true, int ready_rows = 0);
+template <class T>
+int bn_bwd_sums(const T* Y, const T* dO, int upstream, const float* scale, const float* shift, const float* mean,
+                const float* invstd, float* partials, float* sum_g, float* sum_gy, double* dpart, int N, int H, int W, int C,
+                DropoutSpec drop, hipStream_t st, int ready_rows = 0);
 template <class T>
 int relu_mask(const T* Y, const float* scale, const float* shift, uint8_t* out, int N, int H, int W, int C, hipStream_t st);
 template <class T>
diff --git a/acvae_amd/csrc/conv.hip b/acvae_amd/csrc/conv.hip
--- a/acvae_amd/csrc/conv.hip
+++ b/acvae_amd/csrc/conv.hip
@@ -748,8 +748,8 @@
   }
 }
 
-template <class TY>
-__global__ __launch_bounds__(256) void conv1_first_bwd_kernel(const float* __restrict__ x,
+template <class TY, bool BN>
+__global__ __launch_bounds__(256, 3) void conv1_first_bwd_kernel(const float* __restrict__ x,
                                                               const float* __restrict__ scale0,
                                                               const float* __restrict__ shift0,
                                                               const float* __restrict__ mean0,
@@ -757,13 +757,15 @@
                                                               const float* __restrict__ W1,
                                                               const TY* __restrict__ dY,
                                                               float* __restrict__ dw_part, float* __restrict__ bn_part,
-                                                              int T, int F) {
+                                                              int T, int F, BnBwdApply bn) {
+  static_assert(!BN || std::is_same<TY, float>::value, "the fused BatchNorm backward is an fp32 operand");
   __shared__ float wl[64 * 9];
   __shared__ float patch[(C1_RB + 2) * 66];
   constexpr int D_FLOATS = (C1_RB + 2) * 64 * 9, WACC_FLOATS = 8 * 576;
   __shared__ float scratch[D_FLOATS > WACC_FLOATS ? D_FLOATS : WACC_FLOATS];
   float* D = scratch;
   float (*wacc)[576] = reinterpret_cast<float (*)[576]>(scratch);
+  __shared__ BnBwdQuad bnk[BN ? 16 : 1];
   const int nblk_t = (T + C1_RB - 1) / C1_RB;
   const int n = blockIdx.x / nblk_t, t0 = (blockIdx.x % nblk_t) * C1_RB;
   for (int i = threadIdx.x; i < 64 * 9; i += 256) wl[i] = W1[i];
@@ -774,6 +776,8 @@
     if (t >= 0 && t < T && w >= 0 && w < F) v = x[((long)n * T + t) * F + w] * scale0[w] + shift0[w];
     patch[i] = v;
   }
+  if (BN && threadIdx.x < 16)
+    bnk[threadIdx.x] = bn_bwd_quad(bn.scale, bn.shift, bn.mean, bn.invstd, bn.sum_g, bn.sum_gy, threadIdx.x * 4, bn.invn);
   __syncthreads();
   const int cq = threadIdx.x & 15, pp = threadIdx.x >> 4;
   float wreg[4][9];
@@ -788,20 +792,33 @@
     for (int k = 0; k < 9; ++k) dwacc[c][k] = 0.f;
   constexpr int C1_IT = (C1_RB + 2) * 64 / 16, C1_UN = 4;
   static_assert(C1_IT % C1_UN == 0, "pixel loop is unrolled by four");
-  auto fetch = [&](int it, float4& g) {
+  auto inimg_at = [&](int it) {
+    const int pix = pp + it * 16;
+    const int t = t0 + (pix >> 6) - 1;
+    return t >= 0 && t < T && (pix & 63) < F;
+  };
+  auto fetch = [&](int it, float4& g, float4& y) {
     const int pix = pp + it * 16;
     const int r = pix >> 6, w = pix & 63;
     const int t = t0 + r - 1;
-    g = make_float4(0.f, 0.f, 0.f, 0.f);
-    if (t >= 0 && t < T && w < F) g = load4(dY + (((long)n * T + t) * F + w) * 64 + cq * 4);
+    g = y = make_float4(0.f, 0.f, 0.f, 0.f);
+    if (inimg_at(it)) {
+      const long o = (((long)n * T + t) * F + w) * 64 + cq * 4;
+      g = load4(dY + o);
+      if (BN) y = load4(bn.Y + o);
+    }
   };
-  float4 gq[C1_UN], gn[C1_UN];
-#pragma unroll
-  for (int u = 0; u < C1_UN; ++u) fetch(u, gq[u]);
+  auto operand = [&](int it, float4 g, float4 y) { return BN && inimg_at(it) ? bn_bwd_dz(y, g, bnk[cq]) : g; };
+  float4 gq[C1_UN], gn[C1_UN], yn[C1_UN];
+#pragma unroll
+  for (int u = 0; u < C1_UN; ++u) {
+    fetch(u, gn[u], yn[u]);
+    gq[u] = operand(u, gn[u], yn[u]);
+  }
   for (int it0 = 0; it0 < C1_IT; it0 += C1_UN) {
     if (it0 + C1_UN < C1_IT) {
 #pragma unroll
-      for (int u = 0; u < C1_UN; ++u) fetch(it0 + C1_UN + u, gn[u]);
+      for (int u = 0; u < C1_UN; ++u) fetch(it0 + C1_UN + u, gn[u], yn[u]);
     }
 #pragma unroll
     for (int u = 0; u < C1_UN; ++u) {
@@ -829,7 +846,7 @@
       }
     }
 #pragma unroll
-    for (int u = 0; u < C1_UN; ++u) gq[u] = gn[u];
+    for (int u = 0; u < C1_UN; ++u) gq[u] = operand(it0 + C1_UN + u, gn[u], yn[u]);
   }
   __syncthreads();
   const int w = threadIdx.x & 63, rr = threadIdx.x >> 6;
@@ -1053,21 +1070,8 @@
     const int w = (int)(p % W);
     const long t = p / W;
     const int h = (int)(t % H), n = (int)(t / H);
-    const float4 sc = *reinterpret_cast<const float4*>(scale + c), sh = *reinterpret_cast<const float4*>(shift + c);
-    const float4 mu = *reinterpret_cast<const float4*>(mean + c), is = *reinterpret_cast<const float4*>(invstd + c);
-    const float4 sg = *reinterpret_cast<const float4*>(sum_g + c), sgy = *reinterpret_cast<const float4*>(sum_gy + c);
-    const float4 y = load4(Y + 4 * i);
-    float4 g = upstream4<UP>(dO, drop, n, h, w, c, H, W, C);
-    if (y.x * sc.x + sh.x <= 0.f) g.x = 0.f;
-    if (y.y * sc.y + sh.y <= 0.f) g.y = 0.f;
-    if (y.z * sc.z + sh.z <= 0.f) g.z = 0.f;
-    if (y.w * sc.w + sh.w <= 0.f) g.w = 0.f;
-    float4 o;
-    o.x = sc.x * (g.x - sg.x * invn - ((y.x - mu.x) * is.x) * (sgy.x * invn));
-    o.y = sc.y * (g.y - sg.y * invn - ((y.y - mu.y) * is.y) * (sgy.y * invn));
-    o.z = sc.z * (g.z - sg.z * invn - ((y.z - mu.z) * is.z) * (sgy.z * invn));
-    o.w = sc.w * (g.w - sg.w * invn - ((y.w - mu.w) * is.w) * (sgy.w * invn));
-    store4(dYout + 4 * i, o);
+    const BnBwdQuad k = bn_bwd_quad(scale, shift, mean, invstd, sum_g, sum_gy, c, invn);
+    store4(dYout + 4 * i, bn_bwd_dz(load4(Y + 4 * i), upstream4<UP>(dO, drop, n, h, w, c, H, W, C), k));
   }
 }
 
@@ -1078,24 +1082,8 @@
                                                                  const float* __restrict__ sum_g, const float* __restrict__ sum_gy,
                                                                  T* __restrict__ dYout, long total, int C4, float invn) {
   const long tid = blockIdx.x * 256L + threadIdx.x, stride = gridDim.x * 256L;
-  const int c = (int)(tid % C4) * 4;
-  const float4 sc = *reinterpret_cast<const float4*>(scale + c), sh = *reinterpret_cast<const float4*>(shift + c);
-  const float4 mu = *reinterpret_cast<const float4*>(mean + c), is = *reinterpret_cast<const float4*>(invstd + c);
-  float4 a = *reinterpret_cast<const float4*>(sum_g + c), b = *reinterpret_cast<const float4*>(sum_gy + c);
-  a.x *= invn; a.y *= invn; a.z *= invn; a.w *= invn;
-  b.x *= invn; b.y *= invn; b.z *= invn; b.w *= invn;
-  auto one = [&](float4 y, float4 g) {
-    if (y.x * sc.x + sh.x <= 0.f) g.x = 0.f;
-    if (y.y * sc.y + sh.y <= 0.f) g.y = 0.f;
-    if (y.z * sc.z + sh.z <= 0.f) g.z = 0.f;
-    if (y.w * sc.w + sh.w <= 0.f) g.w = 0.f;
-    float4 o;
-    o.x = sc.x * (g.x - a.x - ((y.x - mu.x) * is.x) * b.x);
-    o.y = sc.y * (g.y - a.y - ((y.y - mu.y) * is.y) * b.y);
-    o.z = sc.z * (g.z - a.z - ((y.z - mu.z) * is.z) * b.z);
-    o.w = sc.w * (g.w - a.w - ((y.w - mu.w) * is.w) * b.w);
-    return o;
-  };
+  const BnBwdQuad k = bn_bwd_quad(scale, shift, mean, invstd, sum_g, sum_gy, (int)(tid % C4) * 4, invn);
+  auto one = [&](float4 y, float4 g) { return bn_bwd_dz(y, g, k); };
   long i = tid;
   for (; i + stride < total; i += 2 * stride) {
     const float4 y0 = load4(Y + 4 * i), g0 = load4(dO + 4 * i);
@@ -1138,11 +1126,7 @@
   for (unsigned i = blockIdx.x * 256u + threadIdx.x; i < total; i += gridDim.x * 256u) {
     const PoolIdx q = pool_idx(i, C4, Wc, Hc);
     const int c = q.c4 * 4;
-    const float4 sc = *reinterpret_cast<const float4*>(scale + c), sh = *reinterpret_cast<const float4*>(shift + c);
-    const float4 mu = *reinterpret_cast<const float4*>(mean + c), is = *reinterpret_cast<const float4*>(invstd + c);
-    float4 a = *reinterpret_cast<const float4*>(sum_g + c), b = *reinterpret_cast<const float4*>(sum_gy + c);
-    a.x *= invn; a.y *= invn; a.z *= invn; a.w *= invn;
-    b.x *= invn; b.y *= invn; b.z *= invn; b.w *= invn;
+    const BnBwdQuad kq = bn_bwd_quad(scale, shift, mean, invstd, sum_g, sum_gy, c, invn);
     const long base = (((long)q.n * H + 2 * q.ho) * W + 2 * q.wo) * C + c;
     const bool hx = 2 * q.ho + 1 < H, wx = 2 * q.wo + 1 < W;
     const long off[4] = {0, (long)C, (long)W * C, (long)W * C + C};
@@ -1152,20 +1136,8 @@
     for (int k = 0; k < 4; ++k) y[k] = ok[k] ? load4(Y + base + off[k]) : make_float4(0.f, 0.f, 0.f, 0.f);
     const float4 gp = pool_upstream(dO, drop, q, Ho, Wo, C);
 #pragma unroll
-    for (int k = 0; k < 4; ++k) {
-      if (!ok[k]) continue;
-      float4 g = gp;
-      if (y[k].x * sc.x + sh.x <= 0.f) g.x = 0.f;
-      if (y[k].y * sc.y + sh.y <= 0.f) g.y = 0.f;
-      if (y[k].z * sc.z + sh.z <= 0.f) g.z = 0.f;
-      if (y[k].w * sc.w + sh.w <= 0.f) g.w = 0.f;
-      float4 o;
-      o.x = sc.x * (g.x - a.x - ((y[k].x - mu.x) * is.x) * b.x);
-      o.y = sc.y * (g.y - a.y - ((y[k].y - mu.y) * is.y) * b.y);
-      o.z = sc.z * (g.z - a.z - ((y[k].z - mu.z) * is.z) * b.z);
-      o.w = sc.w * (g.w - a.w - ((y[k].w - mu.w) * is.w) * b.w);
-      store4(dYout + base + off[k], o);
-    }
+    for (int k = 0; k < 4; ++k)
+      if (ok[k]) store4(dYout + base + off[k], bn_bwd_dz(y[k], gp, kq));
   }
 }
 template <class T>
@@ -1488,17 +1460,24 @@
 template <class TY>
 int conv1_first_bwd(const float* x, const float* scale0, const float* shift0, const float* mean0, const float* invstd0,
                     const float* W1, const TY* dY, float* dw_part, float* bn_part, float* dW1, float* dgamma0,
-                    float* dbeta0, double* dpart, int N, int T, int F, hipStream_t st) {
+                    float* dbeta0, double* dpart, int N, int T, int F, hipStream_t st, const BnBwdApply* bn) {
   if (F != 64) return ACVAE_EUNSUPPORTED;
   const int nb = conv1_first_blocks(N, T);
-  hipLaunchKernelGGL(conv1_first_bwd_kernel<TY>, dim3(nb), dim3(256), 0, st, x, scale0, shift0, mean0, invstd0, W1, dY,
-                     dw_part, bn_part, T, F);
+  if (bn) {
+    if (!std::is_same<TY, float>::value) return ACVAE_EUNSUPPORTED;
+    hipLaunchKernelGGL((conv1_first_bwd_kernel<float, true>), dim3(nb), dim3(256), 0, st, x, scale0, shift0, mean0, invstd0, W1,
+                       (const float*)dY, dw_part, bn_part, T, F, *bn);
+  } else {
+    hipLaunchKernelGGL((conv1_first_bwd_kernel<TY, false>), dim3(nb), dim3(256), 0, st, x, scale0, shift0, mean0, invstd0, W1, dY,
+                       dw_part, bn_part, T, F, BnBwdApply{});
+  }
+  ACVAE_LAUNCH_CHECK();
   ACVAE_TRY(colsum2(dw_part, nb, 576, dpart, dW1, nullptr, 0, st));
   ACVAE_TRY(colsum2(bn_part, nb, 128, dpart, dbeta0, dgamma0, 64, st));
   return ACVAE_OK;
 }
-template int conv1_first_bwd<float>(const float*, const float*, const float*, const float*, const float*, const float*, const float*, float*, float*, float*, float*, float*, double*, int, int, int, hipStream_t);
-template int conv1_first_bwd<bf16_t>(const float*, const float*, const float*, const float*, const float*, const float*, const bf16_t*, float*, float*, float*, float*, float*, double*, int, int, int, hipStream_t);
+template int conv1_first_bwd<float>(const float*, const float*, const float*, const float*, const float*, const float*, const float*, float*, float*, float*, float*, float*, double*, int, int, int, hipStream_t, const BnBwdApply*);
+template int conv1_first_bwd<bf16_t>(const float*, const float*, const float*, const float*, const float*, const float*, const bf16_t*, float*, float*, float*, float*, float*, double*, int, int, int, hipStream_t, const BnBwdApply*);
 
 template <class T>
 int bn_relu_pool(const T* Y, const float* scale, const float* shift, T* P, int N, int H, int W, int C,
@@ -1521,42 +1500,56 @@
   return npl * 32 < 32 ? 32 : npl * 32;
 }
 int bn_bwd_blocks(int N, int H, int W, int C) { return cdiv((long)N * H * W, bnb_pix(C)); }
-template <class T>
-int bn_bwd(const T* Y, const T* dO, int upstream, const float* scale, const float* shift, const float* mean,
-           const float* invstd, float* partials, float* sum_g, float* sum_gy, T* dY, double* dpart, int N, int H,
-           int W, int C, DropoutSpec drop, hipStream_t st, bool batch_stats, int ready_rows) {
+static bool bn_bwd_pool_path(int N, int H, int W, int C) { return (long)N * H * W * C < (1L << 31) && H >= 2 && W >= 2; }
+template <class T>
+int bn_bwd_sums(const T* Y, const T* dO, int upstream, const float* scale, const float* shift, const float* mean,
+                const float* invstd, float* partials, float* sum_g, float* sum_gy, double* dpart, int N, int H, int W, int C,
+                DropoutSpec drop, hipStream_t st, int ready_rows) {
   const int Cc = C < 1024 ? C : 1024;
   if (C % 4 != 0 || 1024 % Cc != 0 || C % Cc != 0) return ACVAE_EUNSUPPORTED;
   if (ready_rows > 0 && upstream != UP_PLAIN) return ACVAE_EINVAL;
   const dim3 rgrid(bn_bwd_blocks(N, H, W, C), C / Cc);
-  const int nb = rgrid.x;
   const size_t shm = 256 * 8 * sizeof(float);
-  const long total = (long)N * H * W * (C / 4);
-#define BN_BWD_LAUNCH(UP_)                                                                                             \
-  hipLaunchKernelGGL((bn_bwd_reduce_kernel<UP_, T>), rgrid, dim3(256), shm, st, Y, dO, scale, shift, mean, invstd, partials, \
-                     N, H, W, C, bnb_pix(C), drop);                                                                       \
-  ACVAE_TRY(colsum2(partials, nb, 2 * C, dpart, sum_g, sum_gy, C, st));         \
-  hipLaunchKernelGGL((bn_bwd_apply_kernel<UP_, T>), dim3(ew_grid(total)), dim3(256), 0, st, Y, dO, scale, shift, mean,  \
-                     invstd, sum_g, sum_gy, dY, N, H, W, C, drop, batch_stats ? 1 : 0)
-  const float invn = batch_stats ? 1.0f / (float)((long)N * H * W) : 0.f;
-  const bool small = (long)N * H * W * C < (1L << 31);
-  if (upstream == UP_POOL && small && H >= 2 && W >= 2) {
+  int rows = (int)rgrid.x;
+  if (ready_rows > 0) {
+    rows = ready_rows;
+  } else if (upstream == UP_POOL && bn_bwd_pool_path(N, H, W, C)) {
     const long wins = (long)N * (H / 2) * (W / 2);
     const int wpb = bnb_pix(C) / 4 > 0 ? bnb_pix(C) / 4 : 1;
     const dim3 pgrid((unsigned)cdiv(wins, wpb), C / Cc);
     hipLaunchKernelGGL((bn_bwd_reduce_pool_kernel<T>), pgrid, dim3(256), shm, st, Y, dO, scale, shift, mean, invstd, partials, N, H, W,
                        C, wpb, drop);
-    ACVAE_TRY(colsum2(partials, (int)pgrid.x, 2 * C, dpart, sum_g, sum_gy, C, st));
+    rows = (int)pgrid.x;
+  } else if (upstream == UP_POOL) {
+    hipLaunchKernelGGL((bn_bwd_reduce_kernel<UP_POOL, T>), rgrid, dim3(256), shm, st, Y, dO, scale, shift, mean, invstd, partials,
+                       N, H, W, C, bnb_pix(C), drop);
+  } else if (upstream == UP_DROP) {
+    hipLaunchKernelGGL((bn_bwd_reduce_kernel<UP_DROP, T>), rgrid, dim3(256), shm, st, Y, dO, scale, shift, mean, invstd, partials,
+                       N, H, W, C, bnb_pix(C), drop);
+  } else {
+    hipLaunchKernelGGL((bn_bwd_reduce_kernel<UP_PLAIN, T>), rgrid, dim3(256), shm, st, Y, dO, scale, shift, mean, invstd, partials,
+                       N, H, W, C, bnb_pix(C), drop);
+  }
+  ACVAE_LAUNCH_CHECK();
+  return colsum2(partials, rows, 2 * C, dpart, sum_g, sum_gy, C, st);
+}
+template <class T>
+int bn_bwd_apply(const T* Y, const T* dO, int upstream, const float* scale, const float* shift, const float* mean,
+                 const float* invstd, const float* sum_g, const float* sum_gy, T* dY, int N, int H, int W, int C,
+                 DropoutSpec drop, hipStream_t st, bool batch_stats) {
+  const float invn = bn_bwd_invn(N, H, W, batch_stats);
+  const long total = (long)N * H * W * (C / 4);
+  if (upstream == UP_POOL && bn_bwd_pool_path(N, H, W, C)) {
     const long totalp = (long)N * ((H + 1) / 2) * ((W + 1) / 2) * (C / 4);
     hipLaunchKernelGGL((bn_bwd_apply_pool_kernel<T>), dim3(ew_grid(totalp)), dim3(256), 0, st, Y, dO, scale, shift, mean, invstd,
                        sum_g, sum_gy, dY, N, H, W, C, drop, invn);
-  } else if (upstream == UP_POOL) { BN_BWD_LAUNCH(UP_POOL); }
-  else if (upstream == UP_DROP) { BN_BWD_LAUNCH(UP_DROP); }
-  else {
-    if (ready_rows <= 0)
-      hipLaunchKernelGGL((bn_bwd_reduce_kernel<UP_PLAIN, T>), rgrid, dim3(256), shm, st, Y, dO, scale, shift, mean, invstd, partials,
-                         N, H, W, C, bnb_pix(C), drop);
-    ACVAE_TRY(colsum2(partials, ready_rows > 0 ? ready_rows : nb, 2 * C, dpart, sum_g, sum_gy, C, st));
+  } else if (upstream == UP_POOL) {
+    hipLaunchKernelGGL((bn_bwd_apply_kernel<UP_POOL, T>), dim3(ew_grid(total)), dim3(256), 0, st, Y, dO, scale, shift, mean,
+                       invstd, sum_g, sum_gy, dY, N, H, W, C, drop, batch_stats ? 1 : 0);
+  } else if (upstream == UP_DROP) {
+    hipLaunchKernelGGL((bn_bwd_apply_kernel<UP_DROP, T>), dim3(ew_grid(total)), dim3(256), 0, st, Y, dO, scale, shift, mean,
+                       invstd, sum_g, sum_gy, dY, N, H, W, C, drop, batch_stats ? 1 : 0);
+  } else {
     int g = ew_grid((total + 1) / 2);
     if ((C / 4) > 256 && (g & 1)) ++g;
     if ((256L * g) % (C / 4) == 0)
@@ -1566,10 +1559,19 @@
       hipLaunchKernelGGL((bn_bwd_apply_kernel<UP_PLAIN, T>), dim3(ew_grid(total)), dim3(256), 0, st, Y, dO, scale, shift, mean,
                          invstd, sum_g, sum_gy, dY, N, H, W, C, drop, batch_stats ? 1 : 0);
   }
-#undef BN_BWD_LAUNCH
-  ACVAE_LAUNCH_CHECK();
-  return ACVAE_OK;
-}
+  ACVAE_LAUNCH_CHECK();
+  return ACVAE_OK;
+}
+template <class T>
+int bn_bwd(const T* Y, const T* dO, int upstream, const float* scale, const float* shift, const float* mean,
+           const float* invstd, float* partials, float* sum_g, float* sum_gy, T* dY, double* dpart, int N, int H,
+           int W, int C, DropoutSpec drop, hipStream_t st, bool batch_stats, int ready_rows) {
+  ACVAE_TRY(bn_bwd_sums(Y, dO, upstream, scale, shift, mean, invstd, partials, sum_g, sum_gy, dpart, N, H, W, C, drop, st,
+                        ready_rows));
+  return bn_bwd_apply(Y, dO, upstream, scale, shift, mean, invstd, sum_g, sum_gy, dY, N, H, W, C, drop, st, batch_stats);
+}
+template int bn_bwd_sums<float>(const float*, const float*, int, const float*, const float*, const float*, const float*, float*, float*, float*, double*, int, int, int, int, DropoutSpec, hipStream_t, int);
+template int bn_bwd_sums<bf16_t>(const bf16_t*, const bf16_t*, int, const float*, const float*, const float*, const float*, float*, float*, float*, double*, int, int, int, int, DropoutSpec, hipStream_t, int);
 template int bn_bwd<float>(const float*, const float*, int, const float*, const float*, const float*, const float*, float*, float*, float*, float*, double*, int, int, int, int, DropoutSpec, hipStream_t, bool, int);
 template int bn_bwd<bf16_t>(const bf16_t*, const bf16_t*, int, const float*, const float*, const float*, const float*, float*, float*, float*, bf16_t*, double*, int, int, int, int, DropoutSpec, hipStream_t, bool, int);
 
diff --git a/acvae_amd/csrc/encoder.hip b/acvae_amd/csrc/encoder.hip
--- a/acvae_amd/csrc/encoder.hip
+++ b/acvae_amd/csrc/encoder.hip
@@ -747,8 +747,13 @@
     ACVAE_TRY(conv_dgrad<TA>((const TA*)dya, P(p_conv(b, 2)), wd_ready ? (TA*)(saved + L.wd2[b]) : wd, dyb, N, H, W, C, C, st, wd_ready,
                              sizeof(TA) == 4 ? &red : nullptr, bnpart, &red_rows));
     DropoutSpec none{0.f, nullptr, 0, 0};
-    ACVAE_TRY(acvae::bn_bwd<TA>(Y1, dyb, UP_PLAIN, n1.scale, n1.shift, n1.mean, n1.invstd, bnpart, G(p_bn(b, 1, 1)),
-                            G(p_bn(b, 1, 0)), dya, dpart, N, H, W, C, none, st, training != 0, red_rows));
+    const bool fold1 = b == 1 && sizeof(TA) == 4;
+    if (fold1)
+      ACVAE_TRY(acvae::bn_bwd_sums<TA>(Y1, dyb, UP_PLAIN, n1.scale, n1.shift, n1.mean, n1.invstd, bnpart, G(p_bn(b, 1, 1)),
+                                       G(p_bn(b, 1, 0)), dpart, N, H, W, C, none, st, red_rows));
+    else
+      ACVAE_TRY(acvae::bn_bwd<TA>(Y1, dyb, UP_PLAIN, n1.scale, n1.shift, n1.mean, n1.invstd, bnpart, G(p_bn(b, 1, 1)),
+                                  G(p_bn(b, 1, 0)), dya, dpart, N, H, W, C, none, st, training != 0, red_rows));
     if (b > 1) {
       ACVAE_TRY(conv_wgrad<TA>((const TA*)dya, (const TA*)(saved + L.p[b - 1]), nullptr, nullptr, G(p_conv(b, 1)), slab, N, H,
                                W, Cin, C, st));
@@ -758,9 +763,12 @@
       TA* t = dp_cur; dp_cur = dp_nxt; dp_nxt = t;
     } else {
       BnPtrs b0 = bn_at(saved, L, 0);
-      ACVAE_TRY(acvae::conv1_first_bwd<TA>(feats, b0.scale, b0.shift, b0.mean, b0.invstd, P(p_conv(1, 1)), (const TA*)dya,
-                                       scratch + L.s_c1w, scratch + L.s_c1b, G(p_conv(1, 1)), G(p_bn0(0)), G(p_bn0(1)),
-                                       dpart, N, T, F, st));
+      const BnBwdApply a1{(const float*)Y1, n1.scale, n1.shift, n1.mean, n1.invstd, G(p_bn(1, 1, 1)), G(p_bn(1, 1, 0)),
+                          bn_bwd_invn(N, H, W, training != 0)};
+      ACVAE_TRY(acvae::conv1_first_bwd<TA>(feats, b0.scale, b0.shift, b0.mean, b0.invstd, P(p_conv(1, 1)),
+                                           fold1 ? (const TA*)dyb : (const TA*)dya, scratch + L.s_c1w, scratch + L.s_c1b,
+                                           G(p_conv(1, 1)), G(p_bn0(0)), G(p_bn0(1)), dpart, N, T, F, st,
+                                           fold1 ? &a1 : nullptr));
     }
     if (block_done) ((void (*)(int, void*))block_done)(b, user);
   }
diff --git a/acvae_amd/csrc/ops_abi.hip b/acvae_amd/csrc/ops_abi.hip
--- a/acvae_amd/csrc/ops_abi.hip
+++ b/acvae_amd/csrc/ops_abi.hip
@@ -226,6 +226,30 @@
   ACVAE_TRY(acvae::colsum_tickets_reset((double*)(ws + L.dpart), (hipStream_t)stream));
   return acvae::conv1_first_bwd(x, bn0, bn0 + 64, bn0 + 128, bn0 + 192, W1_oihw, dY, ws + L.slab, ws + L.slab + nb * 576,
                                 dW1, dgamma0, dbeta0, (double*)(ws + L.dpart), N, T, F, (hipStream_t)stream);
+}
+
+extern "C" int acvae_conv1_first_bwd_bn(const float* x, const float* bn0, const float* W1_oihw, const float* Y1, const float* dO,
+                                        const float* bn1, float* dgamma1, float* dbeta1, float* dW1, float* dgamma0, float* dbeta0,
+                                        void* ws_v, int64_t ws_bytes, int N, int T, int F, int training, void* stream) {
+  if (N <= 0 || T <= 0 || !x || !bn0 || !W1_oihw || !Y1 || !dO || !bn1 || !dgamma1 || !dbeta1 || !dW1 || !dgamma0 || !dbeta0 ||
+      !ws_v)
+    return ACVAE_EINVAL;
+  if (F != 64) return ACVAE_EUNSUPPORTED;
+  const ConvWs L = conv_ws(N, T, F, 1, 64);
+  const long bnpart = al64((long)acvae::bn_bwd_blocks(N, T, F, 64) * 2 * 64);
+  if (ws_bytes < (L.total + bnpart) * 4) return ACVAE_EWORKSPACE;
+  if (!aligned16(ws_v)) return ACVAE_EALIGN;
+  hipStream_t st = (hipStream_t)stream;
+  float* ws = (float*)ws_v;
+  double* dpart = (double*)(ws + L.dpart);
+  const long nb = acvae::conv1_first_blocks(N, T);
+  DropoutSpec none{0.f, nullptr, 0, 0};
+  ACVAE_TRY(acvae::colsum_tickets_reset(dpart, st));
+  ACVAE_TRY(acvae::bn_bwd_sums(Y1, dO, UP_PLAIN, bn1, bn1 + 64, bn1 + 128, bn1 + 192, ws + L.total, dbeta1, dgamma1, dpart, N, T,
+                               F, 64, none, st));
+  const BnBwdApply a1{Y1, bn1, bn1 + 64, bn1 + 128, bn1 + 192, dbeta1, dgamma1, bn_bwd_invn(N, T, F, training != 0)};
+  return acvae::conv1_first_bwd(x, bn0, bn0 + 64, bn0 + 128, bn0 + 192, W1_oihw, dO, ws + L.slab, ws + L.slab + nb * 576, dW1,
+                                dgamma0, dbeta0, dpart, N, T, F, st, &a1);
 }
 
 extern "C" int64_t acvae_bn_workspace_bytes(int N, int H, int W, int C) {
diff --git a/include/acvae_hip.h b/include/acvae_hip.h
--- a/include/acvae_hip.h
+++ b/include/acvae_hip.h
@@ -121,6 +121,9 @@
                         void* ws, int64_t ws_bytes, int N, int H, int W, int Cin, int Cout, void* stream);
 int acvae_conv1_first_bwd(const float* x, const float* bn0, const float* W1_oihw, const float* dY, float* dW1,
                           float* dgamma0, float* dbeta0, void* ws, int64_t ws_bytes, int N, int T, int F, void* stream);
+int acvae_conv1_first_bwd_bn(const float* x, const float* bn0, const float* W1_oihw, const float* Y1, const float* dO,
+                             const float* bn1, float* dgamma1, float* dbeta1, float* dW1, float* dgamma0, float* dbeta0,
+                             void* ws, int64_t ws_bytes, int N, int T, int F, int training, void* stream);
 int acvae_conv3x3_fwd_wino(const float* X, const float* W_oihw, const float* in_scale, const float* in_shift, float* Y,
                            const float* gamma, const float* beta, float* running_mean, float* running_var,
                            int64_t* num_batches_tracked, int training, float* bn_out, void* ws, int64_t ws_bytes, int N,
```

New measurement: 2058, median of 6. 1.02x the previous value.
